# eth-cscs/conflux

Measured on NVIDIA H100. Metric: LU GFLOP/s (FP64, (2/3)N^3), higher is better.
Workload: dtype f64

## Files before the change

conflux_b200/__init__.py:

```python
import ctypes

import numpy as np

from ._lib import ConfluxError, LIB_PATH, SYMBOLS, check, lib

__all__ = ["pinned_empty", "pinned_free", "Comm", "lu_params", "LU_rep", "residual", "validate", "lu_solve", "lu_rcond", "lu_refine", "lu_equilibrate", "lu_svx", "lu_inverse", "lu_det", "timeline", "auto_grid", "lu_dims", "init_matrix_host", "ConfluxError", "dbg", "cholesky", "chol_dims", "chol_auto_grid"]


def auto_grid(M, N, P):
    px, py, pz = ctypes.c_int(), ctypes.c_int(), ctypes.c_int()
    check(lib().cflx_auto_grid(int(M), int(N), int(P), ctypes.byref(px), ctypes.byref(py), ctypes.byref(pz)), "auto_grid")
    return px.value, py.value, pz.value


def lu_dims(M, N, v, Px, Py, Pz):
    o = (ctypes.c_int * 8)()
    check(lib().cflx_lu_dims(int(M), int(N), int(v), int(Px), int(Py), int(Pz), o), "lu_dims")
    return dict(M=o[0], N=o[1], Ml=o[2], Nl=o[3], Nt=o[4], nlayr=o[5], Mt=o[6], P=o[7])


def init_matrix_host(M, N, v, Px, Py, Pz, rank, seed=42, out=None):
    d = lu_dims(M, N, v, Px, Py, Pz)
    if out is None:
        out = np.empty((d["Ml"], d["Nl"]), dtype=np.float64)
# ... 276 lines not shown
    def local_factor(self):
        L = np.empty((self.Ml, self.Nl))
        check(lib().cflx_chol_get_local(self._h, L.ctypes.data), "chol_get_local")
        return L

    def validate(self):
        a, r = ctypes.c_double(), ctypes.c_double()
        check(lib().cflx_chol_validate(self._h, ctypes.byref(a), ctypes.byref(r)), "chol_validate")
        return a.value, r.value

    def solve(self, B):
        B, B2, nrhs = _rhs(self.N, B, "cholesky.solve")
        X = np.empty_like(B2)
        check(lib().cflx_chol_solve(self._h, nrhs, B2.ctypes.data, max(nrhs, 1), X.ctypes.data, max(nrhs, 1)), "chol_solve")
        return X.reshape(B.shape)

    def rcond(self):
        r, a = ctypes.c_double(), ctypes.c_double()
        check(lib().cflx_chol_rcond(self._h, ctypes.byref(r), ctypes.byref(a)), "chol_rcond")
        return r.value, a.value

    def refine(self, B, X, ferr=True):
        shape, B2, X2, nrhs, fe, be = _refine_args(self.N, B, X, "cholesky.refine")
        check(lib().cflx_chol_refine(self._h, nrhs, B2.ctypes.data, nrhs, X2.ctypes.data, nrhs,
                                     fe.ctypes.data if ferr else None, be.ctypes.data), "chol_refine")
        return X2.reshape(shape), (fe if ferr else None), be

    def equilibrate(self, apply=True, upload=True):
        if upload:
            a = np.ascontiguousarray(self.data, dtype=np.float64)
            check(lib().cflx_chol_set_local(self._h, a.ctypes.data), "chol_set_local")
        s = np.zeros(self.N)
        scond, amax, equed, info = ctypes.c_double(), ctypes.c_double(), ctypes.c_char(), ctypes.c_int()
        check(lib().cflx_chol_equilibrate(self._h, 1 if apply else 0, s.ctypes.data, ctypes.byref(scond), ctypes.byref(amax),
                                          ctypes.byref(equed), ctypes.byref(info)), "chol_equilibrate")
        return dict(s=s, scond=scond.value, amax=amax.value, equed=equed.value.decode(), info=info.value)

    def svx(self, B):
        B, B2, nrhs = _rhs(self.N, B, "cholesky.svx")
        X = np.empty_like(B2)
        fe, be = np.empty(nrhs), np.empty(nrhs)
        rcond, equed, info = ctypes.c_double(), ctypes.c_char(), ctypes.c_int()
        check(lib().cflx_chol_svx(self._h, nrhs, B2.ctypes.data, nrhs, X.ctypes.data, nrhs, ctypes.byref(rcond),
                                  fe.ctypes.data, be.ctypes.data, ctypes.byref(equed), ctypes.byref(info)), "chol_svx")
        return X.reshape(B.shape), dict(rcond=rcond.value, ferr=fe, berr=be, equed=equed.value.decode(), info=info.value)

    def inverse(self, out=None):
        ptr, arr = _share_out(out, self.Ml, self.Nl, "cholesky.inverse")
        check(lib().cflx_chol_inverse(self._h, ptr), "chol_inverse")
        return arr

    def det(self, unscaled=False):
        ld, mant, exp = ctypes.c_double(), ctypes.c_double(), ctypes.c_int64()
        check(lib().cflx_chol_det(self._h, 1 if unscaled else 0, ctypes.byref(ld), ctypes.byref(mant), ctypes.byref(exp)),
              "chol_det")
        return dict(logdet=ld.value, mantissa=mant.value, exponent=exp.value)

    def finalize(self, clean=True):
        if self._h:
            lib().cflx_chol_destroy(self._h)
            self._h = ctypes.c_void_p()

    def __del__(self):
        try:
            self.finalize()
        except Exception:
            pass


def chol_dims(N, v, Px, Py, Pz):
    o = (ctypes.c_int * 6)()
    check(lib().cflx_chol_dims(int(N), int(v), int(Px), int(Py), int(Pz), o), "chol_dims")
    return dict(N=o[0], Kappa=o[1], Ml=o[2], Nl=o[3], l=o[4], P=o[5])


def chol_auto_grid(P, N):
    g = (ctypes.c_int * 3)()
    check(lib().cflx_chol_auto_grid(int(P), int(N), g), "chol_auto_grid")
    return tuple(g)


class dbg:

    @staticmethod
    def gemm_tn(AT, B, C=None, alpha=1.0, beta=0.0, reps=1):
        AT = np.asarray(AT, dtype=np.float64)
        B = np.asarray(B, dtype=np.float64)
        K, M = AT.shape
        N = B.shape[1]
        M2, N2 = M + (M & 1), N + (N & 1)
        ATp = np.zeros((K, M2))
        ATp[:, :M] = AT
        Bp = np.zeros((K, N2))
        Bp[:, :N] = B
        Cp = np.zeros((M, N2))
        if C is not None:
            Cp[:, :N] = C
        D, _, ms = dbg.gemm_tn_window(ATp, Bp, Cp, M, N2, K, alpha, beta, in_place=False, reps=reps)
        return D[:, :N], ms

    @staticmethod
    def gemm_tn_window(AT, B, C, M, N, K, alpha=1.0, beta=0.0, at_off=(0, 0), b_off=(0, 0), c_off=(0, 0), in_place=True,
                       reps=1):
        AT = np.ascontiguousarray(AT, dtype=np.float64)
        B = np.ascontiguousarray(B, dtype=np.float64)
        C = np.ascontiguousarray(C, dtype=np.float64)
        D = np.empty_like(C)
        Cout = D if in_place else np.empty_like(C)
        ms = ctypes.c_double()
        check(lib().cflx_dbg_gemm_tn(int(M), int(N), int(K), AT.ctypes.data, AT.shape[0], AT.shape[1],
                                     at_off[0] * AT.shape[1] + at_off[1], B.ctypes.data, B.shape[0], B.shape[1],
                                     b_off[0] * B.shape[1] + b_off[1], C.ctypes.data, C.shape[0], C.shape[1],
                                     int(c_off[0]), int(c_off[1]), float(alpha), float(beta), 1 if in_place else 0,
                                     D.ctypes.data, Cout.ctypes.data, int(reps), ctypes.byref(ms)), "dbg_gemm_tn")
        return D, Cout, ms.value

    @staticmethod
    def gemm_narrow(A, B, C=None, alpha=1.0, beta=0.0, reps=1, out=None):
        A = np.ascontiguousarray(A, dtype=np.float64)
        B = np.ascontiguousarray(B, dtype=np.float64)
        M, K = A.shape
        N = B.shape[1]
        Cp = None
        if C is not None:
            assert C.dtype == np.float64 and C.flags.c_contiguous and C.shape == (M, N)
            Cp = C.ctypes.data
        D = np.empty((M, N)) if out is None else out
        assert D.dtype == np.float64 and D.flags.c_contiguous and D.shape == (M, N)
        ms = ctypes.c_double()
        check(lib().cflx_dbg_gemm_narrow(M, N, K, A.ctypes.data, B.ctypes.data, Cp, float(alpha), float(beta), D.ctypes.data,
                                         int(reps), ctypes.byref(ms)), "dbg_gemm_narrow")
        return D, ms.value

    @staticmethod
    def gemm_narrow_tn(AT, B, C=None, alpha=1.0, beta=0.0, reps=1, out=None):
        AT = np.ascontiguousarray(AT, dtype=np.float64)
        B = np.ascontiguousarray(B, dtype=np.float64)
        K, M = AT.shape
        if B.ndim != 2 or B.shape[0] != K:
            raise ValueError(f"gemm_narrow_tn: B must have {K} rows, got shape {B.shape}")
        N = B.shape[1]
        Cp = None
        if C is not None:
            assert C.dtype == np.float64 and C.flags.c_contiguous and C.shape == (M, N)
            Cp = C.ctypes.data
        D = np.empty((M, N)) if out is None else out
        assert D.dtype == np.float64 and D.flags.c_contiguous and D.shape == (M, N)
        ms = ctypes.c_double()
        check(lib().cflx_dbg_gemm_narrow_tn(M, N, K, AT.ctypes.data, B.ctypes.data, Cp, float(alpha), float(beta),
                                            D.ctypes.data, int(reps), ctypes.byref(ms)), "dbg_gemm_narrow_tn")
        return D, ms.value

    @staticmethod
    def residual(A, mode, v, Kappa=None, grid=(1, 1), pos=(0, 0), Xc=None, Xr=None, reps=1):
        A = np.ascontiguousarray(A, dtype=np.float64)
        Ml, Nl = A.shape
        m = {"nn": 0, "tn": 1, "sym": 2}[mode]
        cvt = lambda X: None if X is None else np.ascontiguousarray(np.asarray(X, dtype=np.float64).reshape(X.shape[0], -1))
        Xc, Xr = cvt(Xc), cvt(Xr)
        nrhs = (Xc if Xc is not None else Xr).shape[1]
        rows = (Ml, Nl, Ml + Nl)[m]
        P, Q = np.empty((rows, nrhs)), np.empty((rows, nrhs))
        ms = ctypes.c_double()
        ptr = lambda a: a.ctypes.data if a is not None else None
        check(lib().cflx_dbg_residual(m, Ml, Nl, A.ctypes.data, int(v), int(Kappa if Kappa is not None else 1 << 30),
                                      int(grid[0]), int(grid[1]), int(pos[0]), int(pos[1]), nrhs, ptr(Xc), ptr(Xr),
                                      P.ctypes.data, Q.ctypes.data, int(reps), ctypes.byref(ms)), "dbg_residual")
        return P, Q, ms.value

    @staticmethod
    def equil(A, v, Kappa=None, grid=(1, 1), pos=(0, 0), M=None, r=None, c=None, equed="N", ncols=None):
        A = np.ascontiguousarray(A, dtype=np.float64)
        Ml, Nl = A.shape
        Px, Py = (int(x) for x in grid)
        M = int(M) if M is not None else (Ml // v) * Px * v
        r = np.ascontiguousarray(np.ones(M) if r is None else r, dtype=np.float64)
        c = np.ascontiguousarray(np.ones(M) if c is None else c, dtype=np.float64)
        out = dict(rowmax=np.empty(M), colmax=np.empty(M), diag=np.empty(M), scaled=np.empty_like(A),
                   sym_scaled=np.empty_like(A), growth=np.empty(2))
        zp = ctypes.c_int()
        check(lib().cflx_dbg_equil(Ml, Nl, int(v), int(Kappa if Kappa is not None else 1 << 30), Px, Py, int(pos[0]),
                                   int(pos[1]), M, A.ctypes.data, r.ctypes.data, c.ctypes.data, equed.encode(),
                                   int(ncols if ncols is not None else M), out["rowmax"].ctypes.data,
                                   out["colmax"].ctypes.data, out["diag"].ctypes.data, out["scaled"].ctypes.data,
                                   out["sym_scaled"].ctypes.data, out["growth"].ctypes.data, ctypes.byref(zp)), "dbg_equil")
        out["zero_pivot"] = zp.value
        return out

    @staticmethod
    def inverse_share(mode, v, grid, pos, M, c0, nc, Ml, Nl, Kappa=None, rows=None, X=None, perm=None, share=None,
                      zero_fill=False):
        m = {"lu": 0, "chol": 1}[mode]
        Px, Py = (int(x) for x in grid)
        ldn = -(-int(nc) // 8) * 8
        W = np.empty((Ml, ldn))
        ptr = lambda a: a.ctypes.data if a is not None else None
        out = Xc = pm = None
        if X is not None and share is not None:
            Xc = np.ascontiguousarray(X, dtype=np.float64)
            out = np.array(share, dtype=np.float64, order="C")
            pm = np.ascontiguousarray(perm, dtype=np.int32) if perm is not None else None
        check(lib().cflx_dbg_inverse_share(m, int(Ml), int(Nl), int(v), int(Kappa if Kappa is not None else 1 << 30), Px, Py,
                                           int(pos[0]), int(pos[1]), int(M), int(c0), int(nc),
                                           int(rows if rows is not None else Ml), ptr(Xc),
                                           Xc.shape[1] if Xc is not None else 0, ptr(pm), W.ctypes.data, ptr(out),
                                           1 if zero_fill else 0), "dbg_inverse_share")
        return W, out

    @staticmethod
    def det(d, s1=None, s2=None, square=False):
        d = np.ascontiguousarray(d, dtype=np.float64).ravel()
        n = d.size
        vec = lambda s: None if s is None else np.ascontiguousarray(s, dtype=np.float64).ravel()
        s1, s2 = vec(s1), vec(s2)
        for s in (s1, s2):
            if s is not None and s.size != n:
                raise ValueError(f"dbg.det: a divisor must have {n} entries, got {s.size}")
        mant, exp, neg, fz, nf = ctypes.c_double(), ctypes.c_int64(), ctypes.c_int(), ctypes.c_int(), ctypes.c_int()
        ptr = lambda a: a.ctypes.data if a is not None else None
        check(lib().cflx_dbg_det(n, d.ctypes.data, ptr(s1), ptr(s2), 1 if square else 0, ctypes.byref(mant),
                                 ctypes.byref(exp), ctypes.byref(neg), ctypes.byref(fz), ctypes.byref(nf)), "dbg_det")
        return dict(mantissa=mant.value, exponent=exp.value, neg=neg.value, first_zero=fz.value, nonfinite=nf.value)

    @staticmethod
    def panel(P, reps=1):
        P = np.ascontiguousarray(P, dtype=np.float64)
        n, v = P.shape
        perm = np.zeros(v, dtype=np.int32)
        A00 = np.zeros((v, v))
        LU = np.zeros((max(n, 1), v))
        ms = ctypes.c_double()
        check(lib().cflx_dbg_panel(n, v, P.ctypes.data, perm.ctypes.data, A00.ctypes.data, LU.ctypes.data, int(reps),
                                   ctypes.byref(ms)), "dbg_panel")
        return perm, A00, LU[:n], ms.value

    @staticmethod
    def trsm(A00, B=None, R=None, nb=0, ld=0):
        A00 = np.ascontiguousarray(A00, dtype=np.float64)
        v = A00.shape[0]
        X = Y = None
        n = B.shape[0] if B is not None else R.shape[1]
        if B is not None:
            B = np.ascontiguousarray(B, dtype=np.float64)
            X = np.empty_like(B)
        if R is not None:
            R = np.ascontiguousarray(R, dtype=np.float64)
            Y = np.empty_like(R)
        check(lib().cflx_dbg_trsm(n, v, int(nb), int(ld), A00.ctypes.data, B.ctypes.data if B is not None else None,
                                  X.ctypes.data if X is not None else None, R.ctypes.data if R is not None else None,
                                  Y.ctypes.data if Y is not None else None), "dbg_trsm")
        return X, Y

    @staticmethod
    def diag_inverse(A00, nb):
        A00 = np.ascontiguousarray(A00, dtype=np.float64)
        v = A00.shape[0]
        Uinv = np.empty((max(v // nb, 1), nb, nb))
        LinvT = np.empty_like(Uinv)
        check(lib().cflx_dbg_diag_inverse(v, int(nb), A00.ctypes.data, Uinv.ctypes.data, LinvT.ctypes.data), "dbg_diag_inverse")
        return Uinv, LinvT

    @staticmethod
    def potrf_tile(A, variant=0):
        A = np.ascontiguousarray(A, dtype=np.float64)
        v = A.shape[0]
        L = np.empty((v, v))
        LT = np.empty((v, v))
        info = ctypes.c_int()
        check(lib().cflx_dbg_potrf_tile(v, A.ctypes.data, L.ctypes.data, LT.ctypes.data, ctypes.byref(info), int(variant)),
              "dbg_potrf_tile")
        return L, LT, info.value

    @staticmethod
    def ozaki_gemm(AT, B, C=None, reps=1, want_planes=False, row0=0, col0=0, max_ctas=0):
        AT = np.ascontiguousarray(AT, dtype=np.float64)
        B = np.ascontiguousarray(B, dtype=np.float64)
        K, Ma = AT.shape
        Nb = B.shape[1]
        M, N = Ma - row0, Nb - col0
        D = np.empty((M, N))
        Cp = np.ascontiguousarray(C, dtype=np.float64) if C is not None else None
        pa = np.zeros((8, Ma, K), dtype=np.int8) if want_planes else None
        pb = np.zeros((8, Nb, K), dtype=np.int8) if want_planes else None
        ea = np.zeros(Ma, dtype=np.int32) if want_planes else None
        eb = np.zeros(Nb, dtype=np.int32) if want_planes else None
        ms, sms = ctypes.c_double(), ctypes.c_double()
        ptr = lambda a: a.ctypes.data if a is not None else None
        check(lib().cflx_dbg_ozaki_gemm(M, N, K, int(row0), int(col0), int(max_ctas), AT.ctypes.data, B.ctypes.data, ptr(Cp),
                                        D.ctypes.data, ptr(pa), ptr(pb), ptr(ea), ptr(eb), int(reps), ctypes.byref(ms),
                                        ctypes.byref(sms)), "dbg_ozaki_gemm")
        return dict(D=D, ms=ms.value, split_ms=sms.value, pa=pa, pb=pb, ea=ea, eb=eb)

    @staticmethod
    def push_pivots(A, pivot_rows, fnpr):
        A = np.array(A, dtype=np.float64, order="C")
        piv = np.ascontiguousarray(pivot_rows, dtype=np.int32)
        gri = np.zeros(A.shape[0], dtype=np.int32)
        a01 = np.zeros((max(1, len(piv)), A.shape[1]))
        check(lib().cflx_dbg_push_pivots(A.shape[0], A.shape[1], A.ctypes.data, len(piv), piv.ctypes.data, int(fnpr),
                                         gri.ctypes.data, a01.ctypes.data), "dbg_push_pivots")
        return A, gri, a01[:len(piv)]

    @staticmethod
    def wgmma_peak(n):
        t = ctypes.c_double()
        check(lib().cflx_dbg_wgmma_peak(int(n), ctypes.byref(t)), "dbg_wgmma_peak")
        return t.value

    @staticmethod
    def fp64_peak_ex(which):
        a, b = ctypes.c_double(), ctypes.c_double()
        check(lib().cflx_dbg_fp64_peak_ex(int(which), ctypes.byref(a), ctypes.byref(b)), "dbg_fp64_peak_ex")
        return a.value, b.value

    @staticmethod
    def fp64_peak(which):
        tf = ctypes.c_double()
        check(lib().cflx_dbg_fp64_peak(int(which), ctypes.byref(tf)), "dbg_fp64_peak")
        return tf.value
```

conflux_b200/_lib.py:

```python
import ctypes
import os

_HERE = os.path.dirname(os.path.abspath(__file__))
LIB_PATH = os.path.join(_HERE, "libconflux_b200.so")
_lib = None

c_double_p = ctypes.POINTER(ctypes.c_double)
c_int_p = ctypes.POINTER(ctypes.c_int)


class ConfluxError(RuntimeError):
    pass


SYMBOLS = [
    "cflx_last_error", "cflx_version", "cflx_device_count", "cflx_get_unique_id", "cflx_comm_create",
    "cflx_comm_barrier", "cflx_comm_destroy", "cflx_host_alloc", "cflx_host_free", "cflx_auto_grid", "cflx_lu_dims", "cflx_init_matrix_host",
    "cflx_lu_create", "cflx_lu_info", "cflx_lu_set_local", "cflx_lu_queue_next_local", "cflx_lu_factor", "cflx_lu_get_factors",
    "cflx_lu_get_permutation", "cflx_lu_residual", "cflx_lu_validate", "cflx_lu_solve", "cflx_lu_solve_trans", "cflx_lu_rcond", "cflx_lu_refine", "cflx_lu_equilibrate", "cflx_lu_svx", "cflx_lu_inverse", "cflx_lu_det", "cflx_lu_launch_count", "cflx_lu_uses_ozaki", "cflx_lu_set_profiling", "cflx_lu_phase_ms", "cflx_lu_timeline",
    "cflx_lu_set_kernel_timing", "cflx_lu_trailing_stats", "cflx_lu_destroy", "cflx_chol_auto_grid", "cflx_chol_auto_tile", "cflx_chol_dims", "cflx_chol_init_matrix_host",
    "cflx_chol_create", "cflx_chol_info", "cflx_chol_set_local", "cflx_chol_factor", "cflx_chol_get_local", "cflx_chol_validate",
    "cflx_chol_solve", "cflx_chol_rcond", "cflx_chol_refine", "cflx_chol_equilibrate", "cflx_chol_svx", "cflx_chol_inverse", "cflx_chol_det", "cflx_chol_launch_count", "cflx_chol_destroy", "cflx_dbg_gemm_tn", "cflx_dbg_gemm_narrow", "cflx_dbg_gemm_narrow_tn", "cflx_dbg_residual", "cflx_dbg_equil", "cflx_dbg_inverse_share", "cflx_dbg_det", "cflx_dbg_panel", "cflx_dbg_trsm", "cflx_dbg_diag_inverse", "cflx_dbg_potrf_tile", "cflx_dbg_push_pivots", "cflx_dbg_ozaki_gemm", "cflx_dbg_wgmma_peak", "cflx_dbg_fp64_peak", "cflx_dbg_fp64_peak_ex",
]


def _preload_nccl():
    import sys
    for d in sys.path:
        cand = os.path.join(d, "nvidia", "nccl", "lib", "libnccl.so.2")
        if os.path.exists(cand):
            try:
                ctypes.CDLL(cand, mode=ctypes.RTLD_GLOBAL)
                return cand
            except OSError:
                pass
    return None


def lib():
    global _lib
    if _lib is None:
        if not os.path.exists(LIB_PATH):
            raise ConfluxError(
                f"{LIB_PATH} is missing: build it with `python -c 'import __graft_entry__ as g; g.build()'` "
                "(conflux_b200 has no CPU fallback)")
        _preload_nccl()
        L = ctypes.CDLL(LIB_PATH)
        L.cflx_last_error.restype = ctypes.c_char_p
        L.cflx_version.restype = ctypes.c_char_p
        L.cflx_comm_destroy.restype = None
        L.cflx_lu_destroy.restype = None
        L.cflx_comm_destroy.argtypes = [ctypes.c_void_p]
        L.cflx_lu_destroy.argtypes = [ctypes.c_void_p]
        L.cflx_comm_barrier.argtypes = [ctypes.c_void_p]
        L.cflx_comm_create.argtypes = [ctypes.c_int, ctypes.c_int, ctypes.c_void_p, ctypes.c_int,
                                       ctypes.POINTER(ctypes.c_void_p)]
        L.cflx_lu_create.argtypes = [ctypes.c_void_p] + [ctypes.c_int] * 6 + [ctypes.POINTER(ctypes.c_void_p)]
        L.cflx_host_alloc.argtypes = [ctypes.c_size_t, ctypes.POINTER(ctypes.c_void_p)]
        L.cflx_host_free.argtypes = [ctypes.c_void_p]
        L.cflx_lu_info.argtypes = [ctypes.c_void_p, c_int_p]
        L.cflx_lu_set_local.argtypes = [ctypes.c_void_p, ctypes.c_void_p]
        L.cflx_lu_queue_next_local.argtypes = [ctypes.c_void_p, ctypes.c_void_p]
        L.cflx_lu_factor.argtypes = [ctypes.c_void_p, c_double_p]
        L.cflx_lu_get_factors.argtypes = [ctypes.c_void_p, ctypes.c_void_p, ctypes.c_void_p]
        L.cflx_lu_get_permutation.argtypes = [ctypes.c_void_p, ctypes.c_void_p]
        L.cflx_lu_residual.argtypes = [ctypes.c_void_p, c_double_p]
        L.cflx_lu_validate.argtypes = [ctypes.c_void_p, c_double_p, c_double_p]
        L.cflx_lu_solve.argtypes = [ctypes.c_void_p, ctypes.c_int, ctypes.c_void_p, ctypes.c_int, ctypes.c_void_p, ctypes.c_int]
        L.cflx_lu_solve_trans.argtypes = [ctypes.c_void_p, ctypes.c_int, ctypes.c_void_p, ctypes.c_int, ctypes.c_void_p,
                                          ctypes.c_int]
        L.cflx_lu_rcond.argtypes = [ctypes.c_void_p, c_double_p, c_double_p]
        L.cflx_lu_refine.argtypes = [ctypes.c_void_p, ctypes.c_int, ctypes.c_int, ctypes.c_void_p, ctypes.c_int, ctypes.c_void_p,
                                     ctypes.c_int, ctypes.c_void_p, ctypes.c_void_p]
        L.cflx_lu_equilibrate.argtypes = [ctypes.c_void_p, ctypes.c_int] + [ctypes.c_void_p] * 7
        L.cflx_lu_svx.argtypes = [ctypes.c_void_p, ctypes.c_int, ctypes.c_int, ctypes.c_void_p, ctypes.c_int, ctypes.c_void_p,
                                  ctypes.c_int] + [ctypes.c_void_p] * 6
        L.cflx_lu_inverse.argtypes = [ctypes.c_void_p, ctypes.c_void_p, c_int_p]
        L.cflx_lu_det.argtypes = [ctypes.c_void_p, ctypes.c_int] + [ctypes.c_void_p] * 5
        L.cflx_lu_uses_ozaki.argtypes = [ctypes.c_void_p]
        L.cflx_lu_launch_count.argtypes = [ctypes.c_void_p, ctypes.POINTER(ctypes.c_int64), ctypes.c_int]
        L.cflx_lu_set_profiling.argtypes = [ctypes.c_void_p, ctypes.c_int]
        L.cflx_lu_phase_ms.argtypes = [ctypes.c_void_p, c_double_p]
        L.cflx_lu_timeline.argtypes = [ctypes.c_void_p, ctypes.c_char_p, ctypes.c_int]
        L.cflx_lu_set_kernel_timing.argtypes = [ctypes.c_void_p, ctypes.c_int]
        L.cflx_lu_trailing_stats.argtypes = [ctypes.c_void_p, c_double_p, c_double_p]
        L.cflx_chol_destroy.restype = None
        L.cflx_chol_destroy.argtypes = [ctypes.c_void_p]
        L.cflx_chol_auto_grid.argtypes = [ctypes.c_int, ctypes.c_int, c_int_p]
        L.cflx_chol_auto_tile.argtypes = [ctypes.c_int] * 3
        L.cflx_chol_dims.argtypes = [ctypes.c_int] * 5 + [c_int_p]
        L.cflx_chol_init_matrix_host.argtypes = [ctypes.c_int] * 6 + [ctypes.c_void_p]
        L.cflx_chol_create.argtypes = [ctypes.c_void_p] + [ctypes.c_int] * 5 + [ctypes.POINTER(ctypes.c_void_p)]
        L.cflx_chol_info.argtypes = [ctypes.c_void_p, c_int_p]
        L.cflx_chol_set_local.argtypes = [ctypes.c_void_p, ctypes.c_void_p]
        L.cflx_chol_factor.argtypes = [ctypes.c_void_p, c_double_p]
        L.cflx_chol_get_local.argtypes = [ctypes.c_void_p, ctypes.c_void_p]
        L.cflx_chol_validate.argtypes = [ctypes.c_void_p, c_double_p, c_double_p]
        L.cflx_chol_solve.argtypes = [ctypes.c_void_p, ctypes.c_int, ctypes.c_void_p, ctypes.c_int, ctypes.c_void_p, ctypes.c_int]
        L.cflx_chol_rcond.argtypes = [ctypes.c_void_p, c_double_p, c_double_p]
        L.cflx_chol_refine.argtypes = [ctypes.c_void_p, ctypes.c_int, ctypes.c_void_p, ctypes.c_int, ctypes.c_void_p, ctypes.c_int,
                                       ctypes.c_void_p, ctypes.c_void_p]
        L.cflx_chol_equilibrate.argtypes = [ctypes.c_void_p, ctypes.c_int] + [ctypes.c_void_p] * 5
        L.cflx_chol_svx.argtypes = [ctypes.c_void_p, ctypes.c_int, ctypes.c_void_p, ctypes.c_int, ctypes.c_void_p, ctypes.c_int
                                    ] + [ctypes.c_void_p] * 5
        L.cflx_chol_inverse.argtypes = [ctypes.c_void_p, ctypes.c_void_p]
        L.cflx_chol_det.argtypes = [ctypes.c_void_p, ctypes.c_int] + [ctypes.c_void_p] * 3
        L.cflx_chol_launch_count.argtypes = [ctypes.c_void_p, ctypes.POINTER(ctypes.c_int64), ctypes.c_int]
        L.cflx_init_matrix_host.argtypes = [ctypes.c_int] * 8 + [ctypes.c_void_p]
        _buf = [ctypes.c_void_p, ctypes.c_int, ctypes.c_int64]
        L.cflx_dbg_gemm_tn.argtypes = [ctypes.c_int] * 3 + _buf + [ctypes.c_int64] + _buf + [ctypes.c_int64] + _buf + [
            ctypes.c_int] * 2 + [ctypes.c_double] * 2 + [ctypes.c_int, ctypes.c_void_p, ctypes.c_void_p, ctypes.c_int,
                                                          c_double_p]
        L.cflx_dbg_gemm_narrow.argtypes = [ctypes.c_int] * 3 + [ctypes.c_void_p] * 3 + [ctypes.c_double] * 2 + [
            ctypes.c_void_p, ctypes.c_int, c_double_p]
        L.cflx_dbg_gemm_narrow_tn.argtypes = [ctypes.c_int] * 3 + [ctypes.c_void_p] * 3 + [ctypes.c_double] * 2 + [
            ctypes.c_void_p, ctypes.c_int, c_double_p]
        L.cflx_dbg_residual.argtypes = [ctypes.c_int] * 3 + [ctypes.c_void_p] + [ctypes.c_int] * 7 + [ctypes.c_void_p] * 4 + [
            ctypes.c_int, c_double_p]
        L.cflx_dbg_equil.argtypes = [ctypes.c_int] * 9 + [ctypes.c_void_p] * 3 + [ctypes.c_char, ctypes.c_int] + [
            ctypes.c_void_p] * 7
        L.cflx_dbg_inverse_share.argtypes = [ctypes.c_int] * 13 + [ctypes.c_void_p, ctypes.c_int] + [ctypes.c_void_p] * 3 + [
            ctypes.c_int]
        L.cflx_dbg_det.argtypes = [ctypes.c_int] + [ctypes.c_void_p] * 3 + [ctypes.c_int] + [ctypes.c_void_p] * 5
        L.cflx_dbg_panel.argtypes = [ctypes.c_int, ctypes.c_int] + [ctypes.c_void_p] * 4 + [ctypes.c_int, c_double_p]
        L.cflx_dbg_trsm.argtypes = [ctypes.c_int] * 3 + [ctypes.c_int64] + [ctypes.c_void_p] * 5
        L.cflx_dbg_diag_inverse.argtypes = [ctypes.c_int, ctypes.c_int] + [ctypes.c_void_p] * 3
        L.cflx_dbg_potrf_tile.argtypes = [ctypes.c_int] + [ctypes.c_void_p] * 4 + [ctypes.c_int]
        L.cflx_dbg_push_pivots.argtypes = [ctypes.c_int, ctypes.c_int, ctypes.c_void_p, ctypes.c_int, ctypes.c_void_p, ctypes.c_int,
                                           ctypes.c_void_p, ctypes.c_void_p]
        L.cflx_dbg_ozaki_gemm.argtypes = [ctypes.c_int] * 6 + [ctypes.c_void_p] * 8 + [ctypes.c_int, c_double_p, c_double_p]
        L.cflx_dbg_wgmma_peak.argtypes = [ctypes.c_int, c_double_p]
        L.cflx_dbg_fp64_peak.argtypes = [ctypes.c_int, c_double_p]
        L.cflx_dbg_fp64_peak_ex.argtypes = [ctypes.c_int, c_double_p, c_double_p]
        _lib = L
    return _lib


def check(rc, what=""):
    if rc != 0:
        msg = lib().cflx_last_error().decode(errors="replace")
        raise ConfluxError(f"{what} failed with status {rc}: {msg}")
```

conflux_b200/csrc/dbg.cu:

```cuda
#include <algorithm>
#include <climits>
#include <limits>
#include <vector>

#include "../../include/conflux_b200.h"
#include "common.cuh"
#include "kernels.h"
#include "lu_state.h"

using namespace cflx;

namespace {
int check_device() {
    int n = 0;
    if (cudaGetDeviceCount(&n) != cudaSuccess || n == 0) {
        cudaGetLastError();
        set_last_error("no CUDA device visible: conflux_b200 has no CPU fallback");
        return CFLX_ERR_NO_DEVICE;
    }
    return CFLX_OK;
}

template <class Run>
int time_reps(Run&& run, int reps, double* ms_out) {
// ... 254 lines not shown
        CFLX_TRY(vec_out(colmax_out));
    }
    if (diag_out) {
        CFLX_TRY(equil_diag(a, L, vec, 0));
        CFLX_TRY(vec_out(diag_out));
    }
    if (scaled_out) {
        CFLX_CUDA(cudaMemcpy(w, a, sizeof(double) * a_n, cudaMemcpyDeviceToDevice));
        CFLX_TRY(equil_apply(w, L, dr.as<double>(), dc.as<double>(), equed, 0));
        CFLX_CUDA(cudaMemcpy(scaled_out, w, sizeof(double) * a_n, cudaMemcpyDeviceToHost));
    }
    if (sym_scaled_out) {
        CFLX_CUDA(cudaMemcpy(w, a, sizeof(double) * a_n, cudaMemcpyDeviceToDevice));
        CFLX_TRY(equil_sym_apply(w, L, dr.as<double>(), 0));
        CFLX_CUDA(cudaMemcpy(sym_scaled_out, w, sizeof(double) * a_n, cudaMemcpyDeviceToHost));
    }
    if (growth_out) {
        CFLX_TRY(equil_growth(a, a, L, ncols, dg.as<double>(), 0));
        CFLX_CUDA(cudaMemcpy(growth_out, dg.p, sizeof(double) * 2, cudaMemcpyDeviceToHost));
    }
    if (zero_pivot_out) {
        CFLX_TRY(equil_zero_pivot(a, L, dz.as<int>(), 0));
        int z = 0;
        CFLX_CUDA(cudaMemcpy(&z, dz.p, sizeof(int), cudaMemcpyDeviceToHost));
        *zero_pivot_out = z == INT_MAX ? 0 : z;
    }
    CFLX_CUDA(cudaDeviceSynchronize());
    return CFLX_OK;
}

int cflx_dbg_inverse_share(int mode, int Ml, int Nl, int v, int Kappa, int Px, int Py, int pi, int pj, int M, int c0,
                           int nc, int rows, const double* X, int ldx, const int* perm, double* W_out,
                           double* share_inout, int zero_fill) {
    CFLX_TRY(check_device());
    if ((mode != 0 && mode != 1) || Ml < 0 || Nl < 0 || v < 1 || Ml % v || Nl % v || Px < 1 || Py < 1 || pi < 0 ||
        pi >= Px || pj < 0 || pj >= Py || M < (Ml / v) * Px * v || M < (Nl / v) * Py * v || c0 < 0 || nc < 1 ||
        c0 + nc > M || rows < 0 || rows > Ml || (share_inout && (!X || ldx < nc || (mode == 0 && !perm))))
        return CFLX_ERR_ARG;
    const Layout L{M, v, Kappa, Ml, Nl, Px, Py, pi, pj};
    const int ldn = (int)round_up(nc, 8);
    if (W_out) {
        DevBuf dW;
        CFLX_TRY(dW.alloc(sizeof(double) * Ml * ldn));
        CFLX_CUDA(cudaMemset(dW.p, 0, sizeof(double) * Ml * ldn));
        CFLX_TRY(launch_inverse_seed(dW.as<double>(), ldn, L, rows, c0, nc, 0));
        CFLX_CUDA(cudaMemcpy(W_out, dW.p, sizeof(double) * Ml * ldn, cudaMemcpyDeviceToHost));
    }
    if (share_inout) {
        const size_t a_n = (size_t)Ml * Nl;
        DevBuf dA, dX, dp;
        CFLX_TRY(dA.alloc(sizeof(double) * a_n));
        CFLX_TRY(dX.alloc(sizeof(double) * M * ldx));
        CFLX_TRY(dp.alloc(sizeof(int) * M));
        CFLX_CUDA(cudaMemcpy(dA.p, share_inout, sizeof(double) * a_n, cudaMemcpyHostToDevice));
        CFLX_CUDA(cudaMemcpy(dX.p, X, sizeof(double) * M * ldx, cudaMemcpyHostToDevice));
        if (mode == 0) CFLX_CUDA(cudaMemcpy(dp.p, perm, sizeof(int) * M, cudaMemcpyHostToDevice));
        CFLX_TRY(launch_inverse_scatter(mode == 0 ? InvKind::LU : InvKind::Chol, dX.as<double>(), ldx, c0, nc,
                                        mode == 0 ? dp.as<int>() : nullptr, L, dA.as<double>(), 0));
        if (mode == 1 && zero_fill) CFLX_TRY(launch_inverse_zero(L, dA.as<double>(), 0));
        CFLX_CUDA(cudaMemcpy(share_inout, dA.p, sizeof(double) * a_n, cudaMemcpyDeviceToHost));
    }
    CFLX_CUDA(cudaDeviceSynchronize());
    return CFLX_OK;
}

int cflx_dbg_det(int n, const double* d, const double* s1, const double* s2, int square, double* mant_out,
                 int64_t* exp_out, int* neg_out, int* first_zero_out, int* nonfinite_out) {
    CFLX_TRY(check_device());
    if (n < 1 || !d || (square != 0 && square != 1)) return CFLX_ERR_ARG;
    DevBuf dv, dr;
    CFLX_TRY(dv.alloc(sizeof(double) * 3 * (size_t)n));
    CFLX_TRY(dr.alloc(sizeof(DetResult)));
    double* v = dv.as<double>();
    CFLX_CUDA(cudaMemcpy(v, d, sizeof(double) * n, cudaMemcpyHostToDevice));
    if (s1) CFLX_CUDA(cudaMemcpy(v + n, s1, sizeof(double) * n, cudaMemcpyHostToDevice));
    if (s2) CFLX_CUDA(cudaMemcpy(v + 2 * (size_t)n, s2, sizeof(double) * n, cudaMemcpyHostToDevice));
    CFLX_TRY(launch_det(v, s1 ? v + n : nullptr, s2 ? v + 2 * (size_t)n : nullptr, n, square != 0, dr.as<DetResult>(), 0));
    DetResult r{};
    CFLX_CUDA(cudaMemcpy(&r, dr.p, sizeof(r), cudaMemcpyDeviceToHost));
    if (mant_out) *mant_out = r.mant;
    if (exp_out) *exp_out = r.exp;
    if (neg_out) *neg_out = r.neg;
    if (first_zero_out) *first_zero_out = r.first_zero;
    if (nonfinite_out) *nonfinite_out = r.nonfinite;
    return CFLX_OK;
}

int cflx_dbg_residual(int mode, int Ml, int Nl, const double* A, int v, int Kappa, int Px, int Py, int pi, int pj,
                      int nrhs, const double* Xc, const double* Xr, double* P_out, double* Q_out, int reps, double* ms_out) {
    CFLX_TRY(check_device());
    if (mode < 0 || mode > 2 || Ml < 0 || Nl < 0 || (Nl & 1) || v < 4 || (v & 3) || nrhs < 1 || !A || Px < 1 || Py < 1 ||
        pi < 0 || pi >= Px || pj < 0 || pj >= Py || (mode != 1 && !Xc) || (mode != 0 && !Xr))
        return CFLX_ERR_ARG;
    const ResidMode m = mode == 0 ? ResidMode::NN : mode == 1 ? ResidMode::TN : ResidMode::SymLower;
    const int rows = mode == 0 ? Ml : mode == 1 ? Nl : Ml + Nl;
    const size_t a_n = (size_t)Ml * Nl, o_n = (size_t)std::max(rows, 1) * nrhs;
    DevBuf dA, dXc, dXr, dP, dQ;
    CFLX_TRY(dA.alloc(sizeof(double) * a_n));
    CFLX_TRY(dXc.alloc(sizeof(double) * (size_t)Nl * nrhs));
    CFLX_TRY(dXr.alloc(sizeof(double) * (size_t)Ml * nrhs));
    CFLX_TRY(dP.alloc(sizeof(double) * o_n));
    CFLX_TRY(dQ.alloc(sizeof(double) * o_n));
    CFLX_CUDA(cudaMemcpy(dA.p, A, sizeof(double) * a_n, cudaMemcpyHostToDevice));
    if (Xc) CFLX_CUDA(cudaMemcpy(dXc.p, Xc, sizeof(double) * (size_t)Nl * nrhs, cudaMemcpyHostToDevice));
    if (Xr) CFLX_CUDA(cudaMemcpy(dXr.p, Xr, sizeof(double) * (size_t)Ml * nrhs, cudaMemcpyHostToDevice));
    const Layout L{0, v, Kappa, Ml, Nl, Px, Py, pi, pj};
    auto run = [&]() {
        return launch_residual(m, dA.as<double>(), L, dXc.as<double>(), dXr.as<double>(), nrhs, nrhs, dP.as<double>(),
                               dQ.as<double>(), nrhs, 0);
    };
    CFLX_TRY(time_reps(run, reps, ms_out));
    CFLX_CUDA(cudaMemset(dP.p, 0, sizeof(double) * o_n));
    CFLX_CUDA(cudaMemset(dQ.p, 0, sizeof(double) * o_n));
    CFLX_TRY(run());
    if (P_out) CFLX_CUDA(cudaMemcpy(P_out, dP.p, sizeof(double) * (size_t)rows * nrhs, cudaMemcpyDeviceToHost));
    if (Q_out) CFLX_CUDA(cudaMemcpy(Q_out, dQ.p, sizeof(double) * (size_t)rows * nrhs, cudaMemcpyDeviceToHost));
    CFLX_CUDA(cudaDeviceSynchronize());
    return CFLX_OK;
}

int cflx_dbg_panel(int n, int v, const double* panel, int* perm_out, double* A00_out, double* LU_out, int reps,
                   double* ms_out) {
    CFLX_TRY(check_device());
    if (n < 0 || v <= 0) return CFLX_ERR_ARG;
    const int64_t ld = std::max<int64_t>(2, round_up(n, 2));
    std::vector<double> WT((size_t)v * ld, 0.0);
    for (int r = 0; r < n; ++r)
        for (int c = 0; c < v; ++c) WT[(size_t)c * ld + r] = panel[(size_t)r * v + c];
    DevBuf dW, dW0, dA00, dA00T, dperm;
    CFLX_TRY(dW.alloc(sizeof(double) * v * ld));
    CFLX_TRY(dW0.alloc(sizeof(double) * v * ld));
    CFLX_TRY(dA00.alloc(sizeof(double) * v * v));
    CFLX_TRY(dA00T.alloc(sizeof(double) * v * v));
    CFLX_TRY(dperm.alloc(sizeof(int) * 2 * v));
    CFLX_CUDA(cudaMemcpy(dW0.p, WT.data(), sizeof(double) * v * ld, cudaMemcpyHostToDevice));
    CFLX_CUDA(cudaMemset(dA00.p, 0, sizeof(double) * v * v));
    Events<2> ev;
    CFLX_TRY(ev.create());
    PanelWorkspace ws{};
    CFLX_TRY(panel_workspace_create(&ws));
    if (const char* e = getenv("CFLX_PANEL_CTAS")) ws.cta_cap = atoi(e);
    if (reps < 1) reps = 1;
    float total = 0;
    int nb = 0, rc = CFLX_OK;
    for (int r = 0; r < reps + 1 && rc == CFLX_OK; ++r) {
        cudaMemcpyAsync(dW.p, dW0.p, sizeof(double) * v * ld, cudaMemcpyDeviceToDevice, 0);
        cudaEventRecord(ev[0]);
        rc = launch_panel_getrf_a00(dW.as<double>(), ld, n, v, dperm.as<int>(), dA00.as<double>(), &nb, &ws, 0);
        cudaEventRecord(ev[1]);
        if (cudaEventSynchronize(ev[1]) != cudaSuccess) rc = CFLX_ERR_CUDA;
        float ms = 0;
        cudaEventElapsedTime(&ms, ev[0], ev[1]);
        if (r > 0) total += ms;
    }
    if (rc == CFLX_OK && n >= v)
        rc = launch_gather_a00(dW.as<double>(), ld, dperm.as<int>(), v, nb, dA00.as<double>(), dA00T.as<double>(), 0);
    panel_workspace_destroy(&ws);
    if (rc != CFLX_OK) {
        if (rc == CFLX_ERR_CUDA) set_last_error("panel kernel failed: %s", cudaGetErrorString(cudaGetLastError()));
        return rc;
    }
    if (ms_out) *ms_out = total / reps;
    if (perm_out) CFLX_CUDA(cudaMemcpy(perm_out, dperm.p, sizeof(int) * v, cudaMemcpyDeviceToHost));
    if (A00_out) CFLX_CUDA(cudaMemcpy(A00_out, dA00.p, sizeof(double) * v * v, cudaMemcpyDeviceToHost));
    if (LU_out) {
        CFLX_CUDA(cudaMemcpy(WT.data(), dW.p, sizeof(double) * v * ld, cudaMemcpyDeviceToHost));
        for (int r = 0; r < n; ++r)
            for (int c = 0; c < v; ++c) LU_out[(size_t)r * v + c] = WT[(size_t)c * ld + r];
    }
    CFLX_CUDA(cudaDeviceSynchronize());
    return CFLX_OK;
}

int cflx_dbg_trsm(int n, int v, int nb, int64_t ld, const double* A00, const double* B, double* X_out, const double* R,
                  double* Y_out) {
    CFLX_TRY(check_device());
    if (n <= 0 || v <= 0 || v % 4 != 0) return CFLX_ERR_ARG;
    if (nb == 0)
        for (int c : {128, 64, 32, 16, 8, 4})
            if (!nb && v % c == 0) nb = c;
    if (nb != 4 && nb != 8 && nb != 16 && nb != 32 && nb != 64 && nb != 128) return CFLX_ERR_UNSUPPORTED;
    if (v % nb != 0) return CFLX_ERR_ARG;
    if (ld == 0) ld = round_up(n, 2);
    if ((ld & 1) || ld < round_up(n, 2)) return CFLX_ERR_ARG;
    const double nan = std::numeric_limits<double>::quiet_NaN();
    std::vector<double> A00T((size_t)v * v), BT((size_t)v * ld, nan), RT((size_t)v * ld, nan);
    for (int i = 0; i < v; ++i)
        for (int j = 0; j < v; ++j) A00T[(size_t)j * v + i] = A00[(size_t)i * v + j];
    DevBuf dA, dAT, dUinv, dLinvT, dP, dL, dR, dU;
    CFLX_TRY(dA.alloc(8 * (size_t)v * v)); CFLX_TRY(dAT.alloc(8 * (size_t)v * v));
    CFLX_TRY(dUinv.alloc(8 * (size_t)v * v)); CFLX_TRY(dLinvT.alloc(8 * (size_t)v * v));
    CFLX_TRY(dP.alloc(8 * (size_t)v * ld)); CFLX_TRY(dL.alloc(8 * (size_t)v * ld));
    CFLX_TRY(dR.alloc(8 * (size_t)v * ld)); CFLX_TRY(dU.alloc(8 * (size_t)v * ld));
    CFLX_CUDA(cudaMemcpy(dA.p, A00, 8 * (size_t)v * v, cudaMemcpyHostToDevice));
    CFLX_CUDA(cudaMemcpy(dAT.p, A00T.data(), 8 * (size_t)v * v, cudaMemcpyHostToDevice));
    CFLX_TRY(launch_diag_inverses(dA.as<double>(), v, nb, dUinv.as<double>(), dLinvT.as<double>(), 0));
    if (B && X_out) {
        for (int r = 0; r < n; ++r)
            for (int c = 0; c < v; ++c) BT[(size_t)c * ld + r] = B[(size_t)r * v + c];
        CFLX_CUDA(cudaMemcpy(dP.p, BT.data(), 8 * (size_t)v * ld, cudaMemcpyHostToDevice));
        CFLX_CUDA(cudaMemset(dL.p, 0, 8 * (size_t)v * ld));
        CFLX_TRY(trsm_right_upper_T(dA.as<double>(), dUinv.as<double>(), v, nb, dP.as<double>(), dL.as<double>(), ld, n, 0));
        CFLX_CUDA(cudaMemcpy(BT.data(), dL.p, 8 * (size_t)v * ld, cudaMemcpyDeviceToHost));
        for (int r = 0; r < n; ++r)
            for (int c = 0; c < v; ++c) X_out[(size_t)r * v + c] = BT[(size_t)c * ld + r];
    }
    if (R && Y_out) {
        for (int i = 0; i < v; ++i)
            for (int c = 0; c < n; ++c) RT[(size_t)i * ld + c] = R[(size_t)i * n + c];
        CFLX_CUDA(cudaMemcpy(dR.p, RT.data(), 8 * (size_t)v * ld, cudaMemcpyHostToDevice));
        CFLX_CUDA(cudaMemset(dU.p, 0, 8 * (size_t)v * ld));
        CFLX_TRY(trsm_left_lower_unit(dAT.as<double>(), dLinvT.as<double>(), v, nb, dR.as<double>(), dU.as<double>(), ld,
                                      (int)round_up(n, 2), 0));
        CFLX_CUDA(cudaMemcpy(RT.data(), dU.p, 8 * (size_t)v * ld, cudaMemcpyDeviceToHost));
        for (int i = 0; i < v; ++i)
            for (int c = 0; c < n; ++c) Y_out[(size_t)i * n + c] = RT[(size_t)i * ld + c];
    }
    CFLX_CUDA(cudaDeviceSynchronize());
    return CFLX_OK;
}

int cflx_dbg_diag_inverse(int v, int nb, const double* A00, double* Uinv_out, double* LinvT_out) {
    CFLX_TRY(check_device());
    if (v <= 0 || nb <= 0 || v % nb != 0 || !A00) return CFLX_ERR_ARG;
    const size_t vv = (size_t)v * v, blocks = (size_t)v * nb;
    DevBuf dA, dU, dL;
    CFLX_TRY(dA.alloc(8 * vv));
    CFLX_TRY(dU.alloc(8 * blocks));
    CFLX_TRY(dL.alloc(8 * blocks));
    CFLX_CUDA(cudaMemcpy(dA.p, A00, 8 * vv, cudaMemcpyHostToDevice));
    CFLX_TRY(launch_diag_inverses(dA.as<double>(), v, nb, dU.as<double>(), dL.as<double>(), 0));
    if (Uinv_out) CFLX_CUDA(cudaMemcpy(Uinv_out, dU.p, 8 * blocks, cudaMemcpyDeviceToHost));
    if (LinvT_out) CFLX_CUDA(cudaMemcpy(LinvT_out, dL.p, 8 * blocks, cudaMemcpyDeviceToHost));
    CFLX_CUDA(cudaDeviceSynchronize());
    return CFLX_OK;
}

int cflx_dbg_potrf_tile(int v, const double* A, double* L_out, double* LT_out, int* info_out, int variant) {
    CFLX_TRY(check_device());
    if (!A || v < 4 || v > 512 || variant < 0 || variant > 2 || (variant == 1 && v != 128) ||
        (variant == 2 && potrf_tile_scratch(v) == 0))
        return CFLX_ERR_ARG;
    const size_t vv = (size_t)v * v;
    DevBuf dD, dUT, dUc, dQ, dinfo;
    CFLX_TRY(dD.alloc(8 * vv));
    CFLX_TRY(dUT.alloc(8 * vv));
    CFLX_TRY(dUc.alloc(8 * vv));
    CFLX_TRY(dinfo.alloc(sizeof(int)));
    if (variant == 2) CFLX_TRY(dQ.alloc(8 * potrf_tile_scratch(v)));
    CFLX_CUDA(cudaMemcpy(dD.p, A, 8 * vv, cudaMemcpyHostToDevice));
    CFLX_CUDA(cudaMemset(dUT.p, 0, 8 * vv));
    CFLX_CUDA(cudaMemset(dinfo.p, 0, sizeof(int)));
    CFLX_TRY(potrf_setup(v));
    int64_t launches = 0;
    if (variant == 1)
        CFLX_TRY(potrf_block128(dD.as<double>(), v, dUT.as<double>(), v, dUc.as<double>(), dinfo.as<int>(), 0, 0));
    else
        CFLX_TRY(potrf_tile(dD.as<double>(), dUT.as<double>(), dQ.as<double>(), dinfo.as<int>(), 0, v, 0, &launches));
    if (L_out) CFLX_CUDA(cudaMemcpy(L_out, dD.p, 8 * vv, cudaMemcpyDeviceToHost));
    if (LT_out) CFLX_CUDA(cudaMemcpy(LT_out, dUT.p, 8 * vv, cudaMemcpyDeviceToHost));
    if (info_out) CFLX_CUDA(cudaMemcpy(info_out, dinfo.p, sizeof(int), cudaMemcpyDeviceToHost));
    CFLX_CUDA(cudaDeviceSynchronize());
    return CFLX_OK;
}

int cflx_dbg_push_pivots(int n_rows, int n_cols, double* A_inout, int npiv, const int* pivot_rows, int fnpr, int* gri_out,
                         double* a01_out) {
    CFLX_TRY(check_device());
    if (n_rows <= 0 || n_cols <= 0 || (n_cols & 1) || npiv < 0 || npiv > n_rows - fnpr || fnpr < 0) return CFLX_ERR_ARG;
    if (npiv == 0) {
        if (gri_out) for (int i = 0; i < n_rows; ++i) gri_out[i] = i;
        return CFLX_OK;
    }
    const int v = npiv;
    DevBuf dA, dtmp, da01, dplan, dgp, dgri, dgrit, digri;
    CFLX_TRY(dA.alloc(8 * (size_t)n_rows * n_cols));
    CFLX_TRY(dtmp.alloc(8 * (size_t)v * n_cols));
    CFLX_TRY(da01.alloc(8 * (size_t)v * n_cols));
    CFLX_TRY(dplan.alloc(sizeof(int) * (6 * (size_t)v + 8 + n_rows)));
    CFLX_TRY(dgp.alloc(sizeof(int) * v));
    CFLX_TRY(dgri.alloc(sizeof(int) * n_rows));
    CFLX_TRY(dgrit.alloc(sizeof(int) * n_rows));
    CFLX_TRY(digri.alloc(sizeof(int) * n_rows));
    CFLX_CUDA(cudaMemcpy(dA.p, A_inout, 8 * (size_t)n_rows * n_cols, cudaMemcpyHostToDevice));
    CFLX_CUDA(cudaMemcpy(dgp.p, pivot_rows, sizeof(int) * v, cudaMemcpyHostToDevice));
    MovePlan plan{};
    int* pm = dplan.as<int>();
    plan.npiv = pm; plan.nel = pm + 4; pm += 8;
    plan.cur_piv = pm; pm += v;
    plan.order = pm; pm += v;
    plan.slot2piv = pm; pm += v;
    plan.early = pm; pm += v;
    plan.late = pm; pm += 2 * v;
    plan.rowsrc = pm;
    CFLX_TRY(launch_iota_gri(dgri.as<int>(), digri.as<int>(), n_rows, n_rows, 1, 0, 0));
    CFLX_TRY(launch_plan_moves(dgp.as<int>(), v, 1, 0, fnpr, n_rows, digri.as<int>(), plan, 0));
    CFLX_TRY(launch_push_phase1(dA.as<double>(), n_cols, n_cols, 0, plan, v, dtmp.as<double>(), da01.as<double>(), n_cols, 0, 0));
    CFLX_TRY(launch_push_phase2(dA.as<double>(), n_cols, n_cols, 0, plan, v, 0));
    CFLX_TRY(launch_push_phase3(dA.as<double>(), n_cols, n_cols, 0, fnpr, plan, v, dtmp.as<double>(), 0));
    CFLX_TRY(launch_update_gri(dgri.as<int>(), dgrit.as<int>(), digri.as<int>(), plan.rowsrc, fnpr, n_rows, n_rows, 1, 0));
    CFLX_CUDA(cudaMemcpy(A_inout, dA.p, 8 * (size_t)n_rows * n_cols, cudaMemcpyDeviceToHost));
    if (gri_out) CFLX_CUDA(cudaMemcpy(gri_out, dgri.p, sizeof(int) * n_rows, cudaMemcpyDeviceToHost));
    if (a01_out) CFLX_CUDA(cudaMemcpy(a01_out, da01.p, 8 * (size_t)v * n_cols, cudaMemcpyDeviceToHost));
    CFLX_CUDA(cudaDeviceSynchronize());
    return CFLX_OK;
}

int cflx_dbg_ozaki_gemm(int M, int N, int K, int row0, int col0, int max_ctas, const double* AT, const double* B,
                        const double* C, double* D, signed char* planesA_out, signed char* planesB_out, int* ea_out,
                        int* eb_out, int reps, double* ms_out, double* split_ms_out) {
    CFLX_TRY(check_device());
    if (M <= 0 || N <= 0 || K <= 0 || (N & 1) || row0 < 0 || col0 < 0 || max_ctas < 0) return CFLX_ERR_ARG;
    const int Ma = row0 + M, Nb = col0 + N;
    const int64_t ldat = round_up(Ma, 2), ldb = Nb, ldc = N;
    DevBuf dA, dB, dC, dC0;
    CFLX_TRY(dA.alloc(sizeof(double) * K * ldat));
    CFLX_TRY(dB.alloc(sizeof(double) * K * ldb));
    CFLX_TRY(dC.alloc(sizeof(double) * M * ldc));
    CFLX_TRY(dC0.alloc(sizeof(double) * M * ldc));
    CFLX_CUDA(cudaMemset(dA.p, 0, sizeof(double) * K * ldat));
    CFLX_CUDA(cudaMemcpy2D(dA.p, ldat * 8, AT, (size_t)Ma * 8, (size_t)Ma * 8, K, cudaMemcpyHostToDevice));
    CFLX_CUDA(cudaMemcpy(dB.p, B, sizeof(double) * K * ldb, cudaMemcpyHostToDevice));
    if (C) CFLX_CUDA(cudaMemcpy(dC0.p, C, sizeof(double) * M * ldc, cudaMemcpyHostToDevice));
    else CFLX_CUDA(cudaMemset(dC0.p, 0, sizeof(double) * M * ldc));
    Events<3> ev;
    CFLX_TRY(ev.create());
    OzakiWorkspace ws;
    int rc = ozaki_workspace_create(&ws, Ma, Nb, K);
    if (reps < 1) reps = 1;
    float ms = 0, ms_split = 0;
    for (int r = 0; r < reps + 1 && rc == CFLX_OK; ++r) {
        cudaMemcpyAsync(dC.p, dC0.p, sizeof(double) * M * ldc, cudaMemcpyDeviceToDevice, 0);
        cudaEventRecord(ev[0]);
        rc = ozaki_split_a(&ws, dA.as<double>(), ldat, Ma, 0);
        if (!rc && col0 > 0) rc = ozaki_split_b(&ws, dB.as<double>(), ldb, 0, col0, 0);
        if (!rc) rc = ozaki_split_b(&ws, dB.as<double>(), ldb, col0, N, 0);
        cudaEventRecord(ev[1]);
        if (!rc) rc = launch_ozaki_gemm(&ws, M, N, row0, col0, dC.as<double>(), ldc, max_ctas, 0);
        cudaEventRecord(ev[2]);
        if (cudaEventSynchronize(ev[2]) != cudaSuccess) {
            set_last_error("ozaki kernel failed: %s", cudaGetErrorString(cudaGetLastError()));
            rc = CFLX_ERR_CUDA;
        }
        float a = 0, b = 0;
        cudaEventElapsedTime(&a, ev[0], ev[1]);
        cudaEventElapsedTime(&b, ev[1], ev[2]);
        if (r > 0) {
            ms_split += a;
            ms += b;
        }
    }
    if (rc == CFLX_OK) {
        if (D) cudaMemcpy(D, dC.p, sizeof(double) * M * ldc, cudaMemcpyDeviceToHost);
        for (int s = 0; s < 8; ++s) {
            if (planesA_out) cudaMemcpy(planesA_out + (size_t)s * Ma * K, ws.planesA + (size_t)s * ws.cap_a * K, (size_t)Ma * K, cudaMemcpyDeviceToHost);
            if (planesB_out) cudaMemcpy(planesB_out + (size_t)s * Nb * K, ws.planesB + (size_t)s * ws.cap_b * K, (size_t)Nb * K, cudaMemcpyDeviceToHost);
        }
        if (ea_out) cudaMemcpy(ea_out, ws.ea, sizeof(int) * Ma, cudaMemcpyDeviceToHost);
        if (eb_out) cudaMemcpy(eb_out, ws.eb, sizeof(int) * Nb, cudaMemcpyDeviceToHost);
        if (cudaDeviceSynchronize() != cudaSuccess) rc = CFLX_ERR_CUDA;
    }
    ozaki_workspace_destroy(&ws);
    if (ms_out) *ms_out = ms / reps;
    if (split_ms_out) *split_ms_out = ms_split / reps;
    return rc;
}

int cflx_dbg_wgmma_peak(int n, double* tmacs_out) {
    CFLX_TRY(check_device());
    if (!tmacs_out) return CFLX_ERR_ARG;
    return wgmma_peak_probe(n, tmacs_out);
}

}
```

conflux_b200/csrc/gemm.cu:

```cuda
#include <cstdlib>

#include "common.cuh"
#include "kernels.h"

namespace cflx {

namespace {
constexpr int BK = 16, STAGES = 4;

template <int WM, int WN>
struct Cfg {
    static constexpr int BM = 64 * WM, BN = 32 * WN;
    static constexpr int LDA = BM + 4, LDB = BN + 4;
    static constexpr int NCONS = WM * WN, NTHREADS = (NCONS + 1) * 32;
    static constexpr bool STAGE_C = (WM == 2);
    static constexpr int NBAR = 2 * STAGES + (STAGE_C ? WM * STAGES : 0);
    static constexpr size_t SMEM = (size_t)STAGES * BK * (LDA + LDB) * sizeof(double) + NBAR * sizeof(uint64_t);
    static_assert(!STAGE_C || (LDA == LDB && 64 / 16 == STAGES), "one slab per warp row and stage, in both parts");
};

__device__ __forceinline__ double2 ld_c2(const double* p) {
    double2 v;
    asm("ld.global.v2.f64 {%0, %1}, [%2];" : "=d"(v.x), "=d"(v.y) : "l"(p));
    return v;
}

template <int WM, int WN, int MINB>
__global__ void __launch_bounds__(Cfg<WM, WN>::NTHREADS, MINB) gemm_tn_kernel(GemmArgs g) {
    using C = Cfg<WM, WN>;
    constexpr int BM = C::BM, BN = C::BN, LDA = C::LDA, LDB = C::LDB, NCONS = C::NCONS;
    extern __shared__ __align__(128) unsigned char smem_raw[];
    double* sA = reinterpret_cast<double*>(smem_raw);
    double* sB = sA + STAGES * BK * LDA;
    uint64_t* full = reinterpret_cast<uint64_t*>(sB + STAGES * BK * LDB);
    uint64_t* empty = full + STAGES;
    uint64_t* cfull = empty + STAGES;

    const int warp = threadIdx.x >> 5, lane = threadIdx.x & 31;
    const int m0 = blockIdx.y * BM, n0 = blockIdx.x * BN;

    if (threadIdx.x == 0) {
        for (int s = 0; s < STAGES; ++s) {
            mbar_init(&full[s], 1);
            mbar_init(&empty[s], NCONS);
        }
        if constexpr (C::STAGE_C)
            for (int b = 0; b < WM * STAGES; ++b) mbar_init(&cfull[b], 1);
        fence_barrier_init();
    }
    __syncthreads();

    if (warp == NCONS) {
        int wm = g.M - m0;
        wm = wm > BM ? BM : ((wm + 1) & ~1);
        int wn = g.N - n0;
        wn = wn > BN ? BN : ((wn + 1) & ~1);
        const int rr = lane & 15;
        const int nkt = (g.K + BK - 1) / BK;
        const bool use_c = (g.beta != 0.0);
        for (int kt = 0; kt < nkt; ++kt) {
            const int s = kt % STAGES, u = kt / STAGES;
            if (u > 0) mbar_wait(&empty[s], (u - 1) & 1);
            const int rows = min(BK, g.K - kt * BK);
            if (lane == 0) mbar_arrive_expect_tx(&full[s], (uint32_t)(rows * (wm + wn) * sizeof(double)));
            __syncwarp();
            if (rr < rows) {
                const int64_t k = (int64_t)kt * BK + rr;
                if (lane < 16)
                    bulk_g2s(sA + (s * BK + rr) * LDA, g.AT + k * g.ldat + m0, (uint32_t)(wm * sizeof(double)), &full[s]);
                else
                    bulk_g2s(sB + (s * BK + rr) * LDB, g.B + k * g.ldb + n0, (uint32_t)(wn * sizeof(double)), &full[s]);
            }
        }
        if constexpr (C::STAGE_C) {
            if (use_c)
                for (int i = 0; i < STAGES; ++i) {
                    const int s = (nkt + i) % STAGES, kt = nkt + i - STAGES;
                    if (kt >= 0) mbar_wait(&empty[s], (kt / STAGES) & 1);
                    const int wr = lane >> 4, r0 = m0 + 64 * wr + 16 * i;
                    const int rows = max(0, min(16, g.M - r0));
                    uint64_t* bar = &cfull[wr * STAGES + i];
                    if (rr == 0) mbar_arrive_expect_tx(bar, (uint32_t)(rows * wn * sizeof(double)));
                    __syncwarp();
                    if (rr < rows)
                        bulk_g2s(sA + (wr * STAGES + s) * BK * LDA + rr * LDA + 4 * (rr & 1),
                                 g.C + (int64_t)(r0 + rr) * g.ldc + n0, (uint32_t)(wn * sizeof(double)), bar);
                }
        }
        return;
    }

    const int wm_off = (warp / WN) * 64, wn_off = (warp % WN) * 32;
    const int g4 = lane >> 2, t4 = lane & 3;
    double acc[4][4][4];
#pragma unroll
    for (int i = 0; i < 4; ++i)
#pragma unroll
        for (int j = 0; j < 4; ++j) acc[i][j][0] = acc[i][j][1] = acc[i][j][2] = acc[i][j][3] = 0.0;

    int kt = 0;
    for (; kt * BK < g.K; ++kt) {
        const int s = kt % STAGES, u = kt / STAGES;
        mbar_wait(&full[s], u & 1);
        const double* a_s = sA + s * BK * LDA + wm_off + g4;
        const double* b_s = sB + s * BK * LDB + wn_off + g4;
        const int rows = min(BK, g.K - kt * BK);
#pragma unroll
        for (int kk = 0; kk < BK; kk += 8) {
            if (kk < rows) {
                const bool hi = kk + 4 < rows;
                const double* a_k = a_s + (kk + t4) * LDA;
                const double* b_k = b_s + (kk + t4) * LDB;
                double b[4][2];
#pragma unroll
                for (int j = 0; j < 4; ++j) {
                    b[j][0] = b_k[8 * j];
                    b[j][1] = hi ? b_k[4 * LDB + 8 * j] : 0.0;
                }
#pragma unroll
                for (int i = 0; i < 4; ++i) {
                    const double a[4] = {a_k[16 * i], a_k[16 * i + 8], hi ? a_k[4 * LDA + 16 * i] : 0.0,
                                         hi ? a_k[4 * LDA + 16 * i + 8] : 0.0};
#pragma unroll
                    for (int j = 0; j < 4; ++j) dmma16x8x8(acc[i][j], a, b[j]);
                }
            }
        }
        __syncwarp();
        if (lane == 0) mbar_arrive(&empty[s]);
    }

    const double alpha = g.alpha, beta = g.beta;
    const bool use_c = (beta != 0.0);
    const int row0 = m0 + wm_off + g4, col0 = n0 + wn_off + 2 * t4;
    if constexpr (C::STAGE_C) {
        const int wr = warp / WN, nkt = kt;
#pragma unroll
        for (int i = 0; i < 4; ++i) {
            const double* cs = sA + (wr * STAGES + (nkt + i) % STAGES) * BK * LDA + 4 * (g4 & 1) + wn_off + 2 * t4;
            if (use_c) mbar_wait(&cfull[wr * STAGES + i], 0);
#pragma unroll
            for (int h = 0; h < 2; ++h) {
                const int row = row0 + 16 * i + 8 * h;
#pragma unroll
                for (int j = 0; j < 4; ++j) {
                    const int col = col0 + 8 * j;
                    if (row < g.M && col < g.N) {
                        double2 cv = make_double2(0.0, 0.0);
                        if (use_c) cv = *reinterpret_cast<const double2*>(cs + (g4 + 8 * h) * LDA + 8 * j);
                        double2 out;
                        out.x = fma(alpha, acc[i][j][2 * h], beta * cv.x);
                        out.y = fma(alpha, acc[i][j][2 * h + 1], beta * cv.y);
                        *reinterpret_cast<double2*>(g.D + (int64_t)row * g.ldd + col) = out;
                    }
                }
            }
        }
    } else {
#pragma unroll
        for (int sl = 0; sl < 8; ++sl) {
            const int row = row0 + 8 * sl;
            double2 cv[4];
#pragma unroll
            for (int j = 0; j < 4; ++j) {
                const int col = col0 + 8 * j;
                cv[j] = make_double2(0.0, 0.0);
                if (use_c && row < g.M && col < g.N) cv[j] = ld_c2(g.C + (int64_t)row * g.ldc + col);
            }
#pragma unroll
            for (int j = 0; j < 4; ++j) {
                const int col = col0 + 8 * j;
                if (row < g.M && col < g.N) {
                    double2 out;
                    out.x = fma(alpha, acc[sl / 2][j][2 * (sl & 1)], beta * cv[j].x);
                    out.y = fma(alpha, acc[sl / 2][j][2 * (sl & 1) + 1], beta * cv[j].y);
                    *reinterpret_cast<double2*>(g.D + (int64_t)row * g.ldd + col) = out;
                }
            }
        }
    }
}
}

namespace {
template <int WM, int WN, int MINB>
int setup_one() {
    static PerDeviceMax cfg;
    if (cfg.raise(Cfg<WM, WN>::SMEM))
        CFLX_CUDA(cudaFuncSetAttribute(gemm_tn_kernel<WM, WN, MINB>, cudaFuncAttributeMaxDynamicSharedMemorySize,
                                       (int)Cfg<WM, WN>::SMEM));
    return CFLX_OK;
}
template <int WM, int WN, int MINB>
int launch_one(const GemmArgs& g, cudaStream_t stream) {
    using C = Cfg<WM, WN>;
    CFLX_TRY((setup_one<WM, WN, MINB>()));
    dim3 grid((g.N + C::BN - 1) / C::BN, (g.M + C::BM - 1) / C::BM);
    gemm_tn_kernel<WM, WN, MINB><<<grid, C::NTHREADS, C::SMEM, stream>>>(g);
    CFLX_CUDA(cudaGetLastError());
    return CFLX_OK;
}
int tile_variant() {
    static int v = -1;
    if (v < 0) {
        const char* e = getenv("CFLX_GEMM_TILE");
        v = (e && atoi(e) == 64) ? 64 : 128;
    }
    return v;
}
}

int gemm_tn_setup() {
    CFLX_TRY((setup_one<2, 4, 1>()));
    CFLX_TRY((setup_one<1, 4, 2>()));
    return CFLX_OK;
}

int launch_gemm_tn(const GemmArgs& g, cudaStream_t stream) {
    if (g.M <= 0 || g.N <= 0 || g.K <= 0) return CFLX_OK;
    if ((g.K & 3) || (g.N & 1) || (g.ldat & 1) || (g.ldb & 1) || (g.ldc & 1) || (g.ldd & 1)) {
        set_last_error("gemm_tn: unsupported shape M=%d N=%d K=%d ld=(%lld,%lld,%lld,%lld)", g.M, g.N, g.K,
                       (long long)g.ldat, (long long)g.ldb, (long long)g.ldc, (long long)g.ldd);
        return CFLX_ERR_UNSUPPORTED;
    }
    if (tile_variant() == 64) return launch_one<1, 4, 2>(g, stream);
    return launch_one<2, 4, 1>(g, stream);
}

}
```

conflux_b200/csrc/kernels.h:

```cpp
#pragma once
#include <cuda_runtime.h>

#include <cstdint>

namespace cflx {

struct GemmArgs {
    int M, N, K;
    const double* AT;
    int64_t ldat;
    const double* B;
    int64_t ldb;
    const double* C;
    int64_t ldc;
    double* D;
    int64_t ldd;
    double alpha, beta;
};
int gemm_tn_setup();
int launch_gemm_tn(const GemmArgs& g, cudaStream_t stream);

struct OzakiWorkspace {
    struct Maps;
    int8_t* planesA = nullptr;
    int8_t* planesB = nullptr;
    int* ea = nullptr;
    int* eb = nullptr;
    Maps* maps = nullptr;
    int K = 0, cap_a = 0, cap_b = 0, sms = 0;
};
int ozaki_workspace_create(OzakiWorkspace* ws, int max_rows, int max_cols, int K);
void ozaki_workspace_destroy(OzakiWorkspace* ws);
int ozaki_split_a(OzakiWorkspace* ws, const double* LT, int64_t ld, int n, cudaStream_t s);
int ozaki_split_b(OzakiWorkspace* ws, const double* U, int64_t ld, int col0, int n, cudaStream_t s);
int wgmma_peak_probe(int n, double* tmacs_out);
int launch_ozaki_gemm(OzakiWorkspace* ws, int M, int N, int row0, int col0, double* C, int64_t ldc, int max_ctas, cudaStream_t s);

struct PanelWorkspace {
    void* slot_hdr;
    void* slot_rows;
    int epoch;
    int max_ctas;
    int cta_cap;
    unsigned* sk_flags;
    int* sk_ppos;
    unsigned* sk_ticket;
    unsigned sk_epoch, sk_ticket_count;
    int sk_enabled;
};
int panel_workspace_create(PanelWorkspace* ws);
void panel_workspace_destroy(PanelWorkspace* ws);
int launch_panel_getrf(double* W, int64_t ldw, int n, int v, int* perm_out, PanelWorkspace* ws, cudaStream_t stream);
int launch_panel_getrf_a00(double* W, int64_t ldw, int n, int v, int* perm_out, double* A00, int* nb_used,
                           PanelWorkspace* ws, cudaStream_t stream);

int launch_extract_panel_T(const double* A, int64_t lda, int64_t row0, int64_t col0, int n, int v, double* PT,
                           int64_t ldp, cudaStream_t stream);
int launch_store_panel_T(double* A, int64_t lda, int64_t row0, int64_t col0, int n, int v, const double* LT,
                         int64_t ldp, cudaStream_t stream);
int launch_gather_winners(const double* PT, int64_t ldp, const int* tags, int n_valid, const int* perm, int v,
                          double* out_vals, int64_t ldo, int* out_tags, int dst0, cudaStream_t stream);
int launch_gather_a00(const double* W, int64_t ldw, const int* perm, int v, int nb, double* A00, double* A00T,
                      cudaStream_t stream);

struct MovePlan {
    int* npiv;
    int* cur_piv;
    int* order;
    int* slot2piv;
    int* early;
    int* late;
    int* nel;
    int* rowsrc;
};
int launch_plan_moves(const int* gpivots, int v, int Px, int pi, int fnpr, int Ml, const int* igri, MovePlan plan,
                      cudaStream_t stream);
int launch_push_phase1(const double* A, int64_t lda, int ncols, int col_lo, MovePlan plan, int v, double* tmp,
                       double* a01raw, int64_t ld01, int c0, cudaStream_t stream);
int launch_push_phase2(double* A, int64_t lda, int ncols, int col_lo, MovePlan plan, int v, cudaStream_t stream);
int launch_push_phase3(double* A, int64_t lda, int ncols, int col_lo, int fnpr, MovePlan plan, int v,
                       const double* tmp, cudaStream_t stream);
int launch_update_gri(int* gri, int* gri_tmp, int* igri, const int* rowsrc, int fnpr, int Ml, int v, int Px,
                      cudaStream_t stream);
int launch_compact_panel(const double* PT, int64_t ldp, double* PT2, int64_t ldp2, const int* rowsrc, int fnpr_old,
                         const int* npiv, int Ml, int v, cudaStream_t stream);
int launch_store_u_rows(double* A, int64_t lda, int fnpr_old, MovePlan plan, const double* U, int64_t ldu, int c0,
                        int ncols, int v, cudaStream_t stream);
int launch_store_diag(double* A, int64_t lda, int fnpr_old, MovePlan plan, const double* A00, int loff, int v,
                      cudaStream_t stream);
int launch_split_factors(const double* F, int64_t ldf, int n, double* LT, double* U, cudaStream_t stream);
int launch_gather_perm_rows(const double* A, int64_t lda, const int* perm, int n, double* out, cudaStream_t stream);
constexpr int SUMSQ_PARTIALS = 1184;
int launch_sumsq(const double* X, int64_t count, double* out, double* partials, cudaStream_t stream);
int launch_sum_partials(const double* partials, int n, double* out, cudaStream_t stream);
int launch_fill(double* p, int64_t n, double val, cudaStream_t stream);
int launch_iota_gri(int* gri, int* igri, int Ml, int v, int Px, int pi, cudaStream_t stream);
int launch_pack_bcast(const double* A00, const int* tags, int v, double* buf, cudaStream_t stream);
int launch_unpack_bcast(const double* buf, int v, double* A00, double* A00T, int* gpivots, cudaStream_t stream);
int launch_record_pivots(const int* gpivots, int v, int* hist, int k, cudaStream_t stream);

int launch_diag_inverses(const double* A00, int v, int nb, double* Uinv, double* LinvT, cudaStream_t stream);
int trsm_right_upper_T(const double* A00, const double* Uinv, int v, int nb, double* PT, double* LT, int64_t ld,
                       int n, cudaStream_t stream);
int trsm_left_lower_unit(const double* A00T, const double* LinvT, int v, int nb, double* R, double* U, int64_t ld,
                         int n, cudaStream_t stream);

size_t potrf_tile_scratch(int v);
int potrf_setup(int v);
int potrf_tile(double* D, double* UT, double* Q, int* info, int col0, int v, cudaStream_t stream, int64_t* launches);
int potrf_block128(double* D, int ldd, double* UT, int ldu, double* Uc, int* info, int col0, cudaStream_t stream);

int launch_gather_rows(const double* A, int64_t lda, const int* src_rows, int nrows, int ncols, double* out,
                       cudaStream_t stream);

int launch_gemm_narrow(int M, int N, int K, const double* A, int64_t lda, const double* B, int64_t ldb, const double* C,
                       int64_t ldc, double* D, int64_t ldd, double alpha, double beta, cudaStream_t stream);
int launch_gemm_narrow_tn(int M, int N, int K, const double* AT, int64_t ldat, const double* B, int64_t ldb,
                          const double* C, int64_t ldc, double* D, int64_t ldd, double alpha, double beta,
                          cudaStream_t stream);

enum class ResidMode { NN, TN, SymLower };

}
```

conflux_b200/csrc/lu.cu:

```cuda
#include <algorithm>
#include <cmath>
#include <cstdarg>
#include <cstdlib>
#include <cstring>
#include <random>
#include <string>
#include <vector>

#include <nvtx3/nvToolsExt.h>

#include "lu_state.h"

namespace cflx {
static thread_local char g_err[1024] = "";
void set_last_error(const char* fmt, ...) {
    va_list ap;
    va_start(ap, fmt);
    vsnprintf(g_err, sizeof(g_err), fmt, ap);
    va_end(ap);
}
}

using namespace cflx;

namespace {
int flipbit(int n, int k) { return n ^ (1 << k); }
int butterfly_pair(int pi, int r, int Px) {
    int src = flipbit(pi, r);
    if (src >= Px) {
        if (r == 0) src = pi;
        else {
            src = flipbit(src, r - 1);
            if (src >= Px) src = Px - 1;
        }
    }
    return src;
}
#include "init_tables.inc"
bool fixed_input_matrix(int n, std::vector<double>* out) {
    for (const InitTable& t : kInitTables) {
        if (t.n != n) continue;
        out->clear();
        out->reserve((size_t)n * n);
        if (t.kind == 0) {
            for (const char* p = t.text; *p; ++p) out->push_back((double)(*p - '0'));
        } else {
            const char* p = t.text;
            while (*p) {
                char* e = nullptr;
                out->push_back(std::strtod(p, &e));
                p = (*e == ',') ? e + 1 : e;
            }
        }
        return out->size() == (size_t)n * n;
    }
    return false;
}
int pick_nb(int v) {
    static int cap = -1;
    if (cap < 0) {
        const char* e = getenv("CFLX_TRSM_NB");
        cap = e ? atoi(e) : 128;
    }
    for (int nb : {128, 64, 32, 16, 8, 4})
        if (nb <= cap && v % nb == 0) return nb;
    return 0;
}
}

namespace cflx {
int make_sub(cflx_comm* c, int color, int key, int size, SubComm* out) {
    out->size = size;
    out->rank = key;
    out->c = nullptr;
    if (c->world_size == 1) return CFLX_OK;
    CFLX_NCCL(ncclCommSplit(c->world, color, key, &out->c, nullptr));
    int r = -1, s = -1;
    CFLX_NCCL(ncclCommUserRank(out->c, &r));
    CFLX_NCCL(ncclCommCount(out->c, &s));
    if (r != key || s != size) {
        set_last_error("sub-communicator mismatch: rank %d/%d expected %d/%d", r, s, key, size);
        return CFLX_ERR_NCCL;
    }
    return CFLX_OK;
}
int grid_barrier(cflx_comm* c) {
    if (c->world_size > 1)
        CFLX_NCCL(ncclAllReduce(c->d_scratch, c->d_scratch, 1, ncclDouble, ncclSum, c->world, c->stream));
    CFLX_CUDA(cudaStreamSynchronize(c->stream));
    return CFLX_OK;
}
int grid_init(Grid* g, cflx_comm* c, int Px, int Py, int Pz) {
    g->comm = c;
    g->Px = Px; g->Py = Py; g->Pz = Pz; g->P = Px * Py * Pz;
    g->rank = c->world_rank;
    g->pi = g->rank / (Py * Pz);
    g->pj = (g->rank / Pz) % Py;
    g->pk = g->rank % Pz;
    CFLX_TRY(make_sub(c, g->pi * Py + g->pj, g->pk, Pz, &g->k_comm));
    return make_sub(c, g->pj * Pz + g->pk, g->pi, Px, &g->i_comm);
}
void grid_free(Grid* g) {
    for (SubComm* sc : {&g->k_comm, &g->i_comm})
        if (sc->c) ncclCommDestroy(sc->c);
}

int handle_init(Handle* h, const HandleTexts* texts, cflx_comm* c, int Px, int Py, int Pz) {
    h->texts = texts;
    CFLX_TRY(grid_init(h, c, Px, Py, Pz));
    CFLX_TRY(dmalloc(&h->A0, (size_t)h->Ml * h->Nl));
    return dmalloc(&h->A11, (size_t)h->Ml * h->Nl);
}
int handle_update_setup(Handle* h) {
    CFLX_TRY(gemm_tn_setup());
    const char* e = getenv("CFLX_GEMM");
    if (e && !strcmp(e, "ozaki") && h->nlayr % 128 == 0 && h->nlayr <= 512) {
        CFLX_TRY(ozaki_workspace_create(&h->oz, h->Ml, h->Nl, h->nlayr));
        h->use_ozaki = true;
    }
    return CFLX_OK;
}
int handle_side_stream(Handle* h) {
    int lo = 0, hi = 0;
    cudaDeviceGetStreamPriorityRange(&lo, &hi);
    CFLX_CUDA(cudaStreamCreateWithPriority(&h->side, cudaStreamNonBlocking, hi));
    return CFLX_OK;
}
void handle_free(Handle* h) {
    cudaFree(h->A0);
    cudaFree(h->A11);
    solve_cache_free(&h->sv);
    equil_free(&h->eq);
    if (h->use_ozaki) ozaki_workspace_destroy(&h->oz);
    if (h->side) cudaStreamDestroy(h->side);
    grid_free(h);
}
int handle_set_local(Handle* h, const double* host_local) {
    CFLX_CUDA(cudaSetDevice(h->comm->device));
    cudaStream_t s = h->comm->stream;
    CFLX_CUDA(cudaMemcpyAsync(h->A0, host_local, (size_t)h->Ml * h->Nl * sizeof(double), cudaMemcpyHostToDevice, s));
    CFLX_CUDA(cudaStreamSynchronize(s));
    h->have_input = true;
    h->factored = false;
    h->sv.ready = false;
    h->eq.in.equed = 'N';
    return CFLX_OK;
}
int handle_check(const Handle* h, const char* what) {
    if (h->factored) return CFLX_OK;
    set_last_error(h->texts->unfactored, what);
    return CFLX_ERR_STATE;
}
int handle_equil_begin(Handle* h, bool apply) {
    if (!h->have_input) {
        set_last_error("%s", h->texts->no_input);
        return CFLX_ERR_STATE;
    }
    if (apply && h->eq.in.equed != 'N') {
        set_last_error(h->texts->scaled, h->eq.in.equed);
        return CFLX_ERR_STATE;
    }
    CFLX_CUDA(cudaSetDevice(h->comm->device));
    h->factored = false;
    h->sv.ready = false;
    return CFLX_OK;
}
int handle_equil_end(Handle* h, bool apply, int info, char equed, double rowcnd, double colcnd, const double* c) {
    if (apply && info == 0) CFLX_TRY(equil_record_set(&h->eq.in, equed, rowcnd, colcnd, h->eq.qr, c, h->M, h->comm->stream));
    return CFLX_OK;
}
int handle_launch_count(Handle* h, int64_t* count_out, int reset) {
    if (!h || !count_out) return CFLX_ERR_ARG;
    *count_out = h->launches;
    if (reset) h->launches = 0;
    return CFLX_OK;
}
}

namespace {
struct PhaseTimer {
    cflx_lu* lu;
    int rg;
    cudaStream_t st;
    cudaEvent_t a = nullptr, b = nullptr;
    int ev = -1;
    PhaseTimer(cflx_lu* l, int region, cudaStream_t stream) : lu(l), rg(region), st(stream) {
        nvtxRangePushA(region_name(rg));
        if (lu->prof_mode == 1) {
            cudaEventCreate(&a);
            cudaEventCreate(&b);
            cudaEventRecord(a, st);
        } else if (lu->prof_mode == 2) {
            ev = (int)lu->tl_recs.size() * 2;
            while ((int)lu->tl_pool.size() < ev + 2) {
                cudaEvent_t e;
                cudaEventCreate(&e);
                lu->tl_pool.push_back(e);
            }
            lu->tl_recs.push_back({rg, st == lu->comm->stream ? 0 : 1, ev});
            cudaEventRecord(lu->tl_pool[ev], st);
        }
    }
    ~PhaseTimer() {
        if (lu->prof_mode == 1) {
            cudaEventRecord(b, st);
            cudaEventSynchronize(b);
            float ms = 0;
            cudaEventElapsedTime(&ms, a, b);
            lu->phase_ms[region_phase(rg)] += ms;
            lu->region_ms[st == lu->comm->stream ? 0 : 1][rg] += ms;
            lu->region_cnt[st == lu->comm->stream ? 0 : 1][rg]++;
            cudaEventDestroy(a);
            cudaEventDestroy(b);
        } else if (lu->prof_mode == 2) {
            cudaEventRecord(lu->tl_pool[ev + 1], st);
        }
        nvtxRangePop();
    }
};

int tournament_exchange(cflx_lu* lu, int r, int my_half, cudaStream_t s) {
    const int v = lu->v, Px = lu->Px, pi = lu->pi;
    const int src = butterfly_pair(pi, r, Px);
    const int other = 1 - my_half;
    const size_t hv = (size_t)v * v;
    double* mine = lu->candH + my_half * hv;
    double* recv = lu->candH + other * hv;
    int* mine_t = lu->tagsH + my_half * v;
    int* recv_t = lu->tagsH + other * v;
    const bool self = (src == pi);
    if (self) {
        CFLX_CUDA(cudaMemcpyAsync(recv, mine, hv * sizeof(double), cudaMemcpyDeviceToDevice, s));
        CFLX_CUDA(cudaMemcpyAsync(recv_t, mine_t, v * sizeof(int), cudaMemcpyDeviceToDevice, s));
    }
    bool any = !self;
    for (int ppi = 0; ppi < Px && !any; ++ppi) any = (ppi != pi && butterfly_pair(ppi, r, Px) == pi);
    if (!any) return CFLX_OK;
    CFLX_NCCL(ncclGroupStart());
    for (int ppi = 0; ppi < Px; ++ppi) {
        if (ppi == pi || butterfly_pair(ppi, r, Px) != pi) continue;
        const bool mutual = (!self && ppi == src);
        const double* sv = mutual ? mine : lu->candH + hv;
        const int* st = mutual ? mine_t : lu->tagsH + v;
        CFLX_NCCL(ncclSend(sv, hv, ncclDouble, ppi, lu->i_comm.c, s));
        CFLX_NCCL(ncclSend(st, v, ncclInt, ppi, lu->i_comm.c, s));
    }
    if (!self) {
        CFLX_NCCL(ncclRecv(recv, hv, ncclDouble, src, lu->i_comm.c, s));
        CFLX_NCCL(ncclRecv(recv_t, v, ncclInt, src, lu->i_comm.c, s));
    }
    CFLX_NCCL(ncclGroupEnd());
    return CFLX_OK;
}

__global__ void stack_kernel(const double* __restrict__ candH, const int* __restrict__ tagsH, int v, double* __restrict__ S,
                             double* __restrict__ W2, int* __restrict__ tagsS) {
    const int64_t e = (int64_t)blockIdx.x * blockDim.x + threadIdx.x;
    const int64_t tot = (int64_t)2 * v * v;
    if (e < tot) {
        const int c = (int)(e / (2 * v)), hi = (int)(e % (2 * v));
        const int h = hi / v, i = hi % v;
        const double x = candH[(size_t)h * v * v + (size_t)c * v + i];
        S[e] = x;
        W2[e] = x;
    }
    if (e < 2 * v) tagsS[e] = tagsH[e];
}
int panel_phase(cflx_lu* lu, int k, int fnpr, cudaStream_t s) {
    const int v = lu->v, Px = lu->Px, Py = lu->Py, Pz = lu->Pz, Ml = lu->Ml, Nl = lu->Nl;
    const int pi = lu->pi, pj = lu->pj, pk = lu->pk;
    const int loff = (k / Py) * v, pjk = k % Py;
    if (pj != pjk) return CFLX_OK;
    double* A00 = lu->A00 + (size_t)(k & 1) * v * v;
    double* A00T = lu->A00T + (size_t)(k & 1) * v * v;
    const int n_old = Ml - fnpr;
    const int64_t ldk = std::max<int64_t>(2, round_up(n_old, 2));
    int nR = 0;
    while ((1 << nR) < Px) ++nR;
    {
        PhaseTimer t(lu, RG_step0_copy, s);
        CFLX_TRY(launch_extract_panel_T(lu->A11, Nl, fnpr, loff, n_old, v, lu->PT, ldk, s));
        lu->launches++;
    }
    if (Pz > 1 && n_old > 0) {
        PhaseTimer t(lu, RG_step0_reduce, s);
        CFLX_NCCL(ncclReduce(lu->PT, lu->PT, (size_t)v * ldk, ncclDouble, ncclSum, 0, lu->k_comm.c, s));
    }
    if (pk != 0) return CFLX_OK;
    int my_half = 0;
    {
        PhaseTimer t(lu, RG_step1_A10copy, s);
        CFLX_CUDA(cudaMemcpyAsync(lu->W, lu->PT, (size_t)v * ldk * sizeof(double), cudaMemcpyDeviceToDevice, s));
    }
    {
        PhaseTimer t(lu, RG_step1_lup, s);
        int nb_used = 0;
        if (nR == 0) {
            CFLX_TRY(launch_panel_getrf_a00(lu->W, ldk, n_old, v, lu->perm, A00, &nb_used, &lu->pws, s));
            CFLX_TRY(launch_gather_a00(lu->W, ldk, lu->perm, v, nb_used, A00, A00T, s));
            lu->launches += 2;
        } else {
            CFLX_TRY(launch_panel_getrf(lu->W, ldk, n_old, v, lu->perm, &lu->pws, s));
            lu->launches++;
        }
    }
    {
        PhaseTimer t(lu, RG_step1_rowpermute, s);
        int first_partner = flipbit(pi, 0);
        if (first_partner > Px - 1) first_partner = Px - 1;
        my_half = first_partner < pi ? 1 : 0;
        CFLX_TRY(launch_gather_winners(lu->PT, ldk, lu->gri + fnpr, n_old, lu->perm, v,
                                       lu->candH + (size_t)my_half * v * v, v, lu->tagsH + my_half * v, 0, s));
        lu->launches++;
    }
    PhaseTimer t(lu, RG_step1_pivoting, s);
    for (int r = 0; r < nR; ++r) {
        CFLX_TRY(tournament_exchange(lu, r, my_half, s));
        const int64_t tot = (int64_t)2 * v * v;
        stack_kernel<<<(unsigned)((tot + 255) / 256), 256, 0, s>>>(lu->candH, lu->tagsH, v, lu->S, lu->W2, lu->tagsS);
        CFLX_CUDA(cudaGetLastError());
        const bool last = (r == nR - 1);
        int nb_used = 0;
        if (last) {
            CFLX_TRY(launch_panel_getrf_a00(lu->W2, 2 * v, 2 * v, v, lu->perm, A00, &nb_used, &lu->pws, s));
            CFLX_TRY(launch_gather_a00(lu->W2, 2 * v, lu->perm, v, nb_used, A00, A00T, s));
            lu->launches++;
            my_half = 0;
        } else {
            CFLX_TRY(launch_panel_getrf(lu->W2, 2 * v, 2 * v, v, lu->perm, &lu->pws, s));
            my_half = butterfly_pair(pi, r + 1, Px) < pi ? 1 : 0;
        }
        CFLX_TRY(launch_gather_winners(lu->S, 2 * v, lu->tagsS, 2 * v, lu->perm, v, lu->candH + (size_t)my_half * v * v,
                                       v, lu->tagsH + my_half * v, 0, s));
        lu->launches += 3;
    }
    return CFLX_OK;
}

int ozaki_planes_a(cflx_lu* lu, int n_act, int64_t ld2, cudaStream_t s) {
    if (!lu->use_ozaki || n_act <= 0) return CFLX_OK;
    PhaseTimer t(lu, RG_step6_dgemm, s);
    lu->launches++;
    return ozaki_split_a(&lu->oz, lu->LT + (int64_t)lu->pk * lu->nlayr * ld2, ld2, n_act, s);
}
int ozaki_planes_b(cflx_lu* lu, int col0, int n, int64_t ldu, cudaStream_t s) {
    if (!lu->use_ozaki || n <= 0) return CFLX_OK;
    PhaseTimer t(lu, RG_step6_dgemm, s);
    lu->launches++;
    return ozaki_split_b(&lu->oz, lu->U + (int64_t)lu->pk * lu->nlayr * ldu, ldu, col0, n, s);
}

int trailing_gemm(cflx_lu* lu, int k, int part, int fnpr, int n_act, int col_lo, int ncols, int64_t ld2, int64_t ldu,
                  int u_col_off, cudaStream_t s, int max_ctas = 0) {
    if (n_act <= 0 || ncols <= 0) return CFLX_OK;
    PhaseTimer t(lu, RG_step6_dgemm, s);
    GemmArgs g{};
    g.M = n_act;
    g.N = ncols;
    g.K = lu->nlayr;
    g.AT = lu->LT + (int64_t)lu->pk * lu->nlayr * ld2;
    g.ldat = ld2;
    g.B = lu->U + (int64_t)lu->pk * lu->nlayr * ldu + u_col_off;
    g.ldb = ldu;
    g.C = lu->A11 + (int64_t)fnpr * lu->Nl + col_lo;
    g.ldc = lu->Nl;
    g.D = lu->A11 + (int64_t)fnpr * lu->Nl + col_lo;
    g.ldd = lu->Nl;
    g.alpha = -1.0;
    g.beta = 1.0;
    const int e = 4 * k + 2 * part;
    if (lu->time_gemm) CFLX_CUDA(cudaEventRecord(lu->ev[e], s));
    if (lu->use_ozaki) CFLX_TRY(launch_ozaki_gemm(&lu->oz, g.M, g.N, 0, u_col_off, g.D, g.ldd, max_ctas, s));
    else CFLX_TRY(launch_gemm_tn(g, s));
    if (lu->time_gemm) CFLX_CUDA(cudaEventRecord(lu->ev[e + 1], s));
    lu->ev_used[e / 2] = lu->time_gemm;
    lu->gemm_flops += 2.0 * g.M * (double)g.N * g.K;
    lu->launches++;
    return CFLX_OK;
}

int finish_step(cflx_lu* lu, int k, int& fnpr) {
    cudaStream_t s = lu->comm->stream;
    const int v = lu->v, Px = lu->Px, Py = lu->Py, Pz = lu->Pz, Ml = lu->Ml, Nl = lu->Nl;
    const int pi = lu->pi, pj = lu->pj, pk = lu->pk;
    const int loff = (k / Py) * v, pjk = k % Py, pik = k % Px;
    const bool on_col = (pj == pjk), on_row = (pi == pik), layer0 = (pk == 0);
    const int c0 = loff + (pj <= pjk ? v : 0);
    const int ncols = Nl - c0;
    const int fnpr_old = fnpr;
    const int n_old = Ml - fnpr_old;
    const int64_t ldk = std::max<int64_t>(2, round_up(n_old, 2));
    int nR = 0;
    while ((1 << nR) < Px) ++nR;
    double* A00 = lu->A00 + (size_t)(k & 1) * v * v;
    double* A00T = lu->A00T + (size_t)(k & 1) * v * v;
    {
        PhaseTimer t(lu, RG_step1_A00Buff_bcast, s);
        if (lu->P > 1) {
            const int root = (pik * Py + pjk) * Pz;
            if (lu->rank == root) {
                CFLX_TRY(launch_pack_bcast(A00, lu->tagsH, v, lu->bcast, s));
                lu->launches++;
            }
            CFLX_NCCL(ncclBroadcast(lu->bcast, lu->bcast, (size_t)v * v + v, ncclDouble, root, lu->comm->world, s));
            CFLX_TRY(launch_unpack_bcast(lu->bcast, v, A00, A00T, lu->gpivots, s));
            lu->launches++;
        } else {
            CFLX_CUDA(cudaMemcpyAsync(lu->gpivots, lu->tagsH, v * sizeof(int), cudaMemcpyDeviceToDevice, s));
        }
        CFLX_TRY(launch_record_pivots(lu->gpivots, v, lu->hist, k, s));
        lu->launches++;
    }
    {
        PhaseTimer t(lu, RG_step2_pushingpivots, s);
        CFLX_TRY(launch_plan_moves(lu->gpivots, v, Px, pi, fnpr_old, Ml, lu->igri, lu->plan, s));
        lu->launches++;
        if (Px > 1) {
            CFLX_CUDA(cudaMemcpyAsync(lu->h_npiv, lu->plan.npiv, sizeof(int), cudaMemcpyDeviceToHost, s));
            CFLX_CUDA(cudaEventRecord(lu->ev_npiv, s));
        }
        const int col_lo = layer0 ? 0 : loff;
        const int64_t ldu0 = std::max(2, ncols);
        CFLX_TRY(launch_push_phase1(lu->A11, Nl, Nl, col_lo, lu->plan, v, lu->tmp, ncols > 0 ? lu->A01raw : nullptr, ldu0, c0,
                                    s));
        CFLX_TRY(launch_push_phase2(lu->A11, Nl, Nl, col_lo, lu->plan, v, s));
        CFLX_TRY(launch_push_phase3(lu->A11, Nl, Nl, col_lo, fnpr_old, lu->plan, v, lu->tmp, s));
        CFLX_TRY(launch_update_gri(lu->gri, lu->gri_tmp, lu->igri, lu->plan.rowsrc, fnpr_old, Ml, v, Px, s));
        lu->launches += 5;
    }
    const int64_t ldu = std::max(2, ncols);
    const bool fused_l = (nR == 0);
    if (ncols > 0 && Px * Pz > 1) {
        PhaseTimer t(lu, RG_step2_reduce, s);
        CFLX_NCCL(ncclReduce(lu->A01raw, lu->A01raw, (size_t)v * ldu, ncclDouble, ncclSum, pik * Pz, lu->ik_comm.c, s));
    }
    if (layer0 && ((on_col && !fused_l) || on_row)) {
        PhaseTimer t(lu, RG_step5_dtrsm, s);
        CFLX_TRY(launch_diag_inverses(A00, v, lu->nb, lu->Uinv, lu->LinvT, s));
        lu->launches++;
    }
    const bool split_u = (lu->P == 1) && (k + 1 < lu->Nt) && ncols > v;
    const int ncols_a = split_u ? v : ncols;
    if (on_row && layer0 && ncols > 0) {
        PhaseTimer t(lu, RG_step5_dtrsm, s);
        CFLX_TRY(trsm_left_lower_unit(A00T, lu->LinvT, v, lu->nb, lu->A01raw, lu->U, ldu, ncols_a, s));
        lu->launches += 2 * (v / lu->nb) - 1;
    }
    if (Px * Pz > 1 && ncols > 0) {
        PhaseTimer t(lu, RG_step5_comm, s);
        CFLX_NCCL(ncclBroadcast(lu->U, lu->U, (size_t)v * ldu, ncclDouble, pik * Pz, lu->ik_comm.c, s));
    }
    auto store_factors = [&]() -> int {
        if (!layer0) return CFLX_OK;
        PhaseTimer t(lu, RG_storingresults, s);
        if (ncols > 0) {
            CFLX_TRY(launch_store_u_rows(lu->A11, Nl, fnpr_old, lu->plan, lu->U, ldu, c0, ncols, v, s));
            lu->launches++;
        }
        if (on_col) {
            CFLX_TRY(launch_store_diag(lu->A11, Nl, fnpr_old, lu->plan, A00, loff, v, s));
            lu->launches++;
        }
        return CFLX_OK;
    };
    if (!split_u) CFLX_TRY(store_factors());
    int npiv = v;
    if (Px > 1) {
        CFLX_CUDA(cudaEventSynchronize(lu->ev_npiv));
        npiv = *lu->h_npiv;
    }
    if (npiv < 0 || npiv > v || fnpr_old + npiv > Ml) {
        set_last_error("step %d: inconsistent pivot count %d (fnpr %d, Ml %d)", k, npiv, fnpr_old, Ml);
        return CFLX_ERR_STATE;
    }
    fnpr = fnpr_old + npiv;
    const int n_act = Ml - fnpr;
    const int64_t ld2 = std::max<int64_t>(2, round_up(n_act, 2));
    if (on_col && layer0 && n_act > 0) {
        {
            PhaseTimer t(lu, RG_step4_reshuffling, s);
            CFLX_TRY(launch_compact_panel(fused_l ? lu->W : lu->PT, ldk, fused_l ? lu->LT : lu->PT2, ld2, lu->plan.rowsrc,
                                          fnpr_old, lu->plan.npiv, Ml, v, s));
            lu->launches++;
        }
        if (!fused_l) {
            PhaseTimer t(lu, RG_step4_dtrsm, s);
            CFLX_TRY(trsm_right_upper_T(A00, lu->Uinv, v, lu->nb, lu->PT2, lu->LT, ld2, n_act, s));
            lu->launches += 2 * (v / lu->nb) - 1;
        }
        PhaseTimer t(lu, RG_storingresults, s);
        CFLX_TRY(launch_store_panel_T(lu->A11, Nl, fnpr, loff, n_act, v, lu->LT, ld2, s));
        lu->launches++;
    }
    if (Py * Pz > 1 && n_act > 0) {
        PhaseTimer t(lu, RG_step4_comm, s);
        CFLX_NCCL(ncclBroadcast(lu->LT, lu->LT, (size_t)v * ld2, ncclDouble, pjk * Pz, lu->jk_comm.c, s));
    }
    const bool next_col = (k + 1 < lu->Nt) && (pj == (k + 1) % Py);
    CFLX_TRY(ozaki_planes_a(lu, n_act, ld2, s));
    if (n_act > 0) CFLX_TRY(ozaki_planes_b(lu, 0, split_u ? std::min(v, ncols) : ncols, ldu, s));
    if (next_col) {
        const int w = std::min(v, ncols);
        CFLX_TRY(trailing_gemm(lu, k, 0, fnpr, n_act, c0, w, ld2, ldu, 0, s));
        cudaStream_t side = (lu->prof_mode == 1) ? nullptr : lu->side;
        cudaStream_t sp = side ? side : s;
        if (side) {
            CFLX_CUDA(cudaEventRecord(lu->ev_fork, s));
            CFLX_CUDA(cudaStreamWaitEvent(sp, lu->ev_fork, 0));
        }
        CFLX_TRY(panel_phase(lu, k + 1, fnpr, sp));
        if (side) CFLX_CUDA(cudaEventRecord(lu->ev_join, sp));
        if (split_u) {
            PhaseTimer t(lu, RG_step5_dtrsm, s);
            CFLX_TRY(trsm_left_lower_unit(A00T, lu->LinvT, v, lu->nb, lu->A01raw + v, lu->U + v, ldu, ncols - v, s));
            lu->launches += 2 * (v / lu->nb) - 1;
        }
        if (split_u) CFLX_TRY(store_factors());
        if (split_u && n_act > 0) CFLX_TRY(ozaki_planes_b(lu, w, ncols - w, ldu, s));
        const int leave = (side && lu->use_ozaki) ? lu->pws.cta_cap : 0;
        CFLX_TRY(trailing_gemm(lu, k, 1, fnpr, n_act, c0 + w, ncols - w, ld2, ldu, w, s, leave > 0 ? lu->oz.sms - leave : 0));
        if (side) CFLX_CUDA(cudaStreamWaitEvent(s, lu->ev_join, 0));
    } else {
        CFLX_TRY(trailing_gemm(lu, k, 0, fnpr, n_act, c0, ncols, ld2, ldu, 0, s));
    }
    return CFLX_OK;
}

void free_lu(cflx_lu* lu) {
    if (!lu) return;
    cudaSetDevice(lu->comm->device);
    double* dbl[] = {lu->PT, lu->PT2, lu->W, lu->LT, lu->A01raw, lu->U, lu->tmp, lu->A00, lu->A00T, lu->Uinv, lu->LinvT,
                     lu->candH, lu->S, lu->W2, lu->bcast, lu->Cbuf, lu->xbuf};
    for (double* p : dbl) cudaFree(p);
    int* ints[] = {lu->gri, lu->gri_tmp, lu->igri, lu->perm, lu->gpivots, lu->tagsH, lu->tagsS, lu->hist, lu->plan_mem,
                   lu->idx_buf};
    for (int* p : ints) cudaFree(p);
    if (lu->h_npiv) cudaFreeHost(lu->h_npiv);
    if (lu->pws.slot_hdr) panel_workspace_destroy(&lu->pws);
    for (auto& e : lu->ev) cudaEventDestroy(e);
    for (auto& e : lu->tl_pool) cudaEventDestroy(e);
    if (lu->ev_fork) cudaEventDestroy(lu->ev_fork);
    if (lu->ev_join) cudaEventDestroy(lu->ev_join);
    if (lu->ev_npiv) cudaEventDestroy(lu->ev_npiv);
    if (lu->copy) cudaStreamDestroy(lu->copy);
    if (lu->ev_a0_read) cudaEventDestroy(lu->ev_a0_read);
    if (lu->ev_upload) cudaEventDestroy(lu->ev_upload);
    for (SubComm* sc : {&lu->jk_comm, &lu->ik_comm})
        if (sc->c) ncclCommDestroy(sc->c);
    handle_free(lu);
    delete lu;
}

SolveFactor lu_solve_factor(cflx_lu* lu) { return SolveFactor{*lu, lu->Cbuf, lu->Ml, &lu->jk_comm, &lu->ik_comm, lu->Pz}; }

int lu_solve_prepare(cflx_lu* lu) {
    cudaStream_t s = lu->comm->stream;
    const int v = lu->v, Px = lu->Px, Ml = lu->Ml;
    std::vector<int> hist(lu->M);
    CFLX_TRY(cflx_lu_get_permutation(lu, hist.data()));
    if (lu->pk == 0) {
        cudaFree(lu->sv.inv);
        lu->sv.inv = nullptr;
        if (!lu->Cbuf) CFLX_TRY(dmalloc(&lu->Cbuf, (size_t)Ml * lu->Nl));
        int rc = redistribute_pivoted_rows(lu, hist, true, lu->A11, lu->Cbuf);
        cudaFree(lu->xbuf);
        lu->xbuf = nullptr;
        if (rc) return rc;
        CFLX_TRY(solve_inverses(&lu->sv, lu_solve_factor(lu), false));
        if (lu->pj == 0) {
            std::vector<int> rows(Ml, 0);
            for (int q = 0; q < lu->M; ++q) {
                const int k = q / v;
                if (k % Px == lu->pi) rows[(k / Px) * v + q % v] = hist[q];
            }
            CFLX_TRY(solve_set_rows(&lu->sv.rows, rows, s));
        }
    }
    lu->sv.ready = true;
    lu->sv.trans_ready = false;
    return CFLX_OK;
}

int lu_solve_prepare_trans(cflx_lu* lu) {
    cudaStream_t s = lu->comm->stream;
    const int v = lu->v, Px = lu->Px, Py = lu->Py;
    std::vector<int> hist(lu->M);
    CFLX_TRY(cflx_lu_get_permutation(lu, hist.data()));
    std::vector<int> unperm(lu->M);
    for (int q = 0; q < lu->M; ++q) unperm[hist[q]] = q;
    CFLX_TRY(solve_set_rows(&lu->sv.unperm, unperm, s));
    if (lu->pk == 0 && lu->pj == 0) {
        std::vector<int> rows(lu->Ml, 0);
        for (int q = 0; q < lu->M; ++q)
            if ((q / v) % Px == lu->pi) rows[(q / v / Px) * v + q % v] = q;
        CFLX_TRY(solve_set_rows(&lu->sv.rows_id, rows, s));
    }
    if (lu->pk == 0 && lu->pi == 0) {
        std::vector<int> cols(lu->Nl, 0);
        for (int q = 0; q < lu->M; ++q)
            if ((q / v) % Py == lu->pj) cols[(q / v / Py) * v + q % v] = q;
        CFLX_TRY(solve_set_rows(&lu->sv.cols, cols, s));
    }
    lu->sv.trans_ready = true;
    return CFLX_OK;
}

int lu_sweeps(cflx_lu* lu, bool transposed, bool pa, int nrhs, const double* B, int ldb, double* X, int ldx) {
    if (!lu->sv.ready) CFLX_TRY(lu_solve_prepare(lu));
    if ((transposed || pa) && !lu->sv.trans_ready) CFLX_TRY(lu_solve_prepare_trans(lu));
    const SolveFactor f = lu_solve_factor(lu);
    SolveCache* sc = &lu->sv;
    const int ldn = (int)round_up(nrhs, 8);
    CFLX_TRY(solve_cache_grow(sc, f, ldn, true, transposed, transposed));
    if (!transposed) {
        CFLX_TRY(solve_seed(sc, f, ldn, nrhs, B, ldb, SolveSeed{false, pa ? sc->rows_id : sc->rows, lu->Ml, sc->W}));
        CFLX_TRY(solve_row_sweep(sc, f, ldn, true, sc->W, lu->Px, true));
        CFLX_TRY(solve_row_sweep(sc, f, ldn, false, sc->X, 1, false));
        return solve_finish(sc, f, ldn, nrhs, X, ldx);
    }
    CFLX_TRY(solve_seed(sc, f, ldn, nrhs, B, ldb, SolveSeed{true, sc->cols, lu->Nl, sc->Z}));
    CFLX_TRY(solve_col_sweep(sc, f, ldn, true, Tri::UpperT, sc->Z, lu->Py, true));
    CFLX_TRY(solve_col_sweep(sc, f, ldn, false, Tri::UnitLowerT, sc->X, 1, false));
    return solve_finish(sc, f, ldn, nrhs, X, ldx, pa ? nullptr : sc->unperm);
}

const HandleTexts kLuTexts = {
    "%s requested before cflx_lu_factor, or after cflx_lu_set_local without a factorisation",
    "equilibration requested before cflx_lu_set_local",
    "equilibration refused: the input is already scaled (equed = '%c'); upload it again first"};

int lu_check(const cflx_lu* lu, const char* what, bool own_input) {
    CFLX_TRY(handle_check(lu, what));
    if (own_input && lu->a0_is_next) {
        set_last_error("%s refused: the input buffer of the last run was handed to the queued next matrix", what);
        return CFLX_ERR_STATE;
    }
    return CFLX_OK;
}

int lu_rcond(cflx_lu* lu, bool inf, double* rcond_out, double* anorm_out) {
    double anorm = 0.0, ainvnm = 0.0;
    CFLX_TRY(inf ? norminf_grid(*lu, lu->A0, &anorm) : norm1_grid(*lu, lu->A0, false, &anorm));
    if (anorm > 0.0) {
        auto apply = [&](int kase, double* x) { return lu_sweeps(lu, (kase == 2) != inf, true, 1, x, 1, x, 1); };
        CFLX_TRY(estimate_inv_norm1(lu->M, apply, &ainvnm));
    }
    *rcond_out = rcond_from(anorm, ainvnm);
    if (anorm_out) *anorm_out = anorm;
    return CFLX_OK;
}

RefineOp lu_refine_op(cflx_lu* lu, bool t) {
    auto solve = [lu, t](bool tk, int n, const double* b, int lb, double* x, int lx) {
        return lu_sweeps(lu, t != tk, false, n, b, lb, x, lx);
    };
    return RefineOp{*lu, lu->A0, t ? ResidMode::TN : ResidMode::NN, false, solve};
}
}

extern "C" {

const char* cflx_last_error(void) { return g_err; }
const char* cflx_version(void) { return "conflux_b200 0.1 (sm_90a)"; }

int cflx_device_count(int* count) {
    int n = 0;
    cudaError_t e = cudaGetDeviceCount(&n);
    if (e != cudaSuccess) {
        n = 0;
        cudaGetLastError();
    }
    *count = n;
    return CFLX_OK;
}

int cflx_get_unique_id(void* id_out) {
    static_assert(sizeof(ncclUniqueId) == CFLX_UNIQUE_ID_BYTES, "unique id size");
    ncclUniqueId id;
    CFLX_NCCL(ncclGetUniqueId(&id));
    std::memcpy(id_out, &id, sizeof(id));
    return CFLX_OK;
}

int cflx_comm_create(int world_size, int world_rank, const void* unique_id, int device, cflx_comm** out) {
    if (!out || world_size < 1 || world_rank < 0 || world_rank >= world_size) return CFLX_ERR_ARG;
    int ndev = 0;
    cflx_device_count(&ndev);
    if (ndev == 0) {
        set_last_error("no CUDA device visible: conflux_b200 has no CPU fallback");
        return CFLX_ERR_NO_DEVICE;
    }
    if (device < 0 || device >= ndev) {
        set_last_error("device %d out of range (%d visible)", device, ndev);
        return CFLX_ERR_ARG;
    }
    CFLX_CUDA(cudaSetDevice(device));
    auto* c = new cflx_comm;
    c->world_size = world_size;
    c->world_rank = world_rank;
    c->device = device;
    CFLX_CUDA(cudaStreamCreateWithFlags(&c->stream, cudaStreamNonBlocking));
    CFLX_CUDA(cudaMalloc((void**)&c->d_scratch, sizeof(double)));
    CFLX_CUDA(cudaMemset(c->d_scratch, 0, sizeof(double)));
    if (world_size > 1) {
        if (!unique_id) {
            set_last_error("unique_id required for world_size > 1");
            return CFLX_ERR_ARG;
        }
        ncclUniqueId id;
        std::memcpy(&id, unique_id, sizeof(id));
        CFLX_NCCL(ncclCommInitRank(&c->world, world_size, id, world_rank));
    }
    *out = c;
    return CFLX_OK;
}

int cflx_comm_barrier(cflx_comm* c) {
    if (!c) return CFLX_ERR_ARG;
    CFLX_CUDA(cudaSetDevice(c->device));
    return grid_barrier(c);
}

void cflx_comm_destroy(cflx_comm* c) {
    if (!c) return;
    cudaSetDevice(c->device);
    if (c->world) ncclCommDestroy(c->world);
    if (c->stream) cudaStreamDestroy(c->stream);
    cudaFree(c->d_scratch);
    delete c;
}

int cflx_auto_grid(int M, int N, int P, int* Px, int* Py, int* Pz) {
    if (M <= 0 || N <= 0 || P <= 0) return CFLX_ERR_ARG;
    const double ratio = 1.0 * std::max(M, N) / std::min(M, N);
    const int p1 = (int)std::cbrt(P / ratio);
    const int psq = (int)std::sqrt(P / ratio);
    const int phs = (int)std::sqrt(P / (2 * ratio));
    if (P == psq * psq) {
        *Px = psq; *Py = psq; *Pz = 1;
        return CFLX_OK;
    }
    if (phs * phs == P / 2) {
        *Px = phs; *Py = phs; *Pz = 2;
        return CFLX_OK;
    }
    int d[3] = {p1, (int)(ratio * p1), 0};
    d[2] = P / (d[0] * d[1]);
    std::sort(d, d + 3, [](int a, int b) { return a > b; });
    *Px = d[0]; *Py = d[1]; *Pz = d[2];
    return CFLX_OK;
}

int cflx_lu_dims(int M, int N, int v, int Px, int Py, int Pz, int* o) {
    if (M <= 0 || N <= 0 || v <= 0 || Px <= 0 || Py <= 0 || Pz <= 0 || !o) return CFLX_ERR_ARG;
    const int tx = (int)std::ceil((double)M / (v * Px)), ty = (int)std::ceil((double)N / (v * Py));
    const int Mp = v * Px * tx, Np = v * Py * ty;
    const int Nt = (int)std::ceil((double)Np / v), Mt = (int)std::ceil((double)Mp / v);
    o[0] = Mp; o[1] = Np;
    o[2] = (int)std::ceil((double)Mt / Px) * v;
    o[3] = (int)std::ceil((double)Nt / Py) * v;
    o[4] = Nt; o[5] = (v + Pz - 1) / Pz; o[6] = Mt; o[7] = Px * Py * Pz;
    return CFLX_OK;
}

int cflx_init_matrix_host(int M, int N, int v, int Px, int Py, int Pz, int rank, int seed, double* out) {
    int d[8];
    CFLX_TRY(cflx_lu_dims(M, N, v, Px, Py, Pz, d));
    const int Ml = d[2], Nl = d[3];
    if (rank < 0 || rank >= d[7] || !out) return CFLX_ERR_ARG;
    std::fill(out, out + (size_t)Ml * Nl, 0.0);
    if (rank % Pz != 0) return CFLX_OK;
    if (d[0] == d[1]) {
        std::vector<double> tab;
        if (fixed_input_matrix(d[0], &tab)) {
            const int n = d[0];
            const Layout L{n, v, d[4], Ml, Nl, Px, Py, rank / (Py * Pz), (rank / Pz) % Py};
            for (int lr = 0; lr < Ml; ++lr)
                for (int lc = 0; lc < Nl; ++lc) out[(size_t)lr * Nl + lc] = tab[(size_t)L.row(lr) * n + L.col(lc)];
            return CFLX_OK;
        }
    }
    std::mt19937_64 eng((unsigned long long)(seed + rank));
    std::uniform_real_distribution<double> dist;
    for (int lti = 0; lti < Ml / v; ++lti)
        for (int ltj = 0; ltj < Nl / v; ++ltj)
            for (int li = 0; li < v; ++li)
                for (int lj = 0; lj < v; ++lj) out[(size_t)(lti * v + li) * Nl + ltj * v + lj] = 5 + dist(eng);
    return CFLX_OK;
}

int cflx_lu_create(cflx_comm* c, int M, int N, int v, int Px, int Py, int Pz, cflx_lu** out) {
    if (!c || !out || M <= 0 || N <= 0 || v <= 0) return CFLX_ERR_ARG;
    CFLX_CUDA(cudaSetDevice(c->device));
    if (Px <= 0 || Py <= 0 || Pz <= 0) CFLX_TRY(cflx_auto_grid(M, N, c->world_size, &Px, &Py, &Pz));
    if (Px != Py) {
        set_last_error("grid %dx%dx%d: the CONFLUX LU path requires Px == Py (SURVEY.md fact 6)", Px, Py, Pz);
        return CFLX_ERR_UNSUPPORTED;
    }
    if (Px * Py * Pz != c->world_size) {
        set_last_error("grid %dx%dx%d does not match the %d ranks of the communicator", Px, Py, Pz, c->world_size);
        return CFLX_ERR_ARG;
    }
    if (v % 4 != 0 || v % Pz != 0 || (v / Pz) % 4 != 0 || pick_nb(v) == 0) {
        set_last_error("tile size v=%d unsupported: need v %% 4 == 0 and (v / Pz) %% 4 == 0", v);
        return CFLX_ERR_UNSUPPORTED;
    }
    int d[8];
    CFLX_TRY(cflx_lu_dims(M, N, v, Px, Py, Pz, d));
    if (d[0] != d[1]) {
        set_last_error("only square matrices are supported (the miniapp passes M = N)");
        return CFLX_ERR_UNSUPPORTED;
    }
    auto* lu = new cflx_lu;
    lu->M = d[0]; lu->N = d[1]; lu->Ml = d[2]; lu->Nl = d[3]; lu->Nt = d[4]; lu->nlayr = d[5]; lu->Mt = d[6];
    lu->v = v;
    lu->nb = pick_nb(v);
    int rc = CFLX_OK;
    auto fail = [&](int code) {
        free_lu(lu);
        return code;
// ... 408 lines not shown
```

conflux_b200/csrc/rows.cu:

```cuda
#include <algorithm>

#include "common.cuh"
#include "kernels.h"

namespace cflx {

namespace {

__global__ void extract_panel_T_kernel(const double* __restrict__ A, int64_t lda, int64_t row0, int64_t col0, int n,
                                       int v, double* __restrict__ PT, int64_t ldp) {
    __shared__ double tile[32][33];
    const int r0 = blockIdx.x * 32, c0 = blockIdx.y * 32;
    for (int dy = threadIdx.y; dy < 32; dy += blockDim.y) {
        const int r = r0 + dy, c = c0 + threadIdx.x;
        if (r < n && c < v) tile[dy][threadIdx.x] = A[(row0 + r) * lda + col0 + c];
    }
    __syncthreads();
    for (int dy = threadIdx.y; dy < 32; dy += blockDim.y) {
        const int c = c0 + dy, r = r0 + threadIdx.x;
        if (r < n && c < v) PT[(int64_t)c * ldp + r] = tile[threadIdx.x][dy];
    }
}
__global__ void store_panel_T_kernel(double* __restrict__ A, int64_t lda, int64_t row0, int64_t col0, int n, int v,
                                     const double* __restrict__ LT, int64_t ldp) {
    __shared__ double tile[32][33];
    const int r0 = blockIdx.x * 32, c0 = blockIdx.y * 32;
    for (int dy = threadIdx.y; dy < 32; dy += blockDim.y) {
        const int c = c0 + dy, r = r0 + threadIdx.x;
        if (r < n && c < v) tile[dy][threadIdx.x] = LT[(int64_t)c * ldp + r];
    }
    __syncthreads();
    for (int dy = threadIdx.y; dy < 32; dy += blockDim.y) {
        const int r = r0 + dy, c = c0 + threadIdx.x;
        if (r < n && c < v) A[(row0 + r) * lda + col0 + c] = tile[threadIdx.x][dy];
    }
}

__global__ void gather_winners_kernel(const double* __restrict__ PT, int64_t ldp, const int* __restrict__ tags,
                                      int n_valid, const int* __restrict__ perm, int v, double* __restrict__ out,
                                      int64_t ldo, int* __restrict__ out_tags, int dst0) {
    const int64_t e = (int64_t)blockIdx.x * blockDim.x + threadIdx.x;
    if (e >= (int64_t)v * v) return;
    const int c = (int)(e / v), i = (int)(e % v);
    const int src = perm[i];
    out[(int64_t)c * ldo + dst0 + i] = src < n_valid ? PT[(int64_t)c * ldp + src] : 0.0;
    if (c == 0) out_tags[dst0 + i] = src < n_valid ? tags[src] : 0;
}
__global__ void gather_a00_kernel(const double* __restrict__ W, int64_t ldw, const int* __restrict__ perm, int v, int nb,
                                  double* __restrict__ A00, double* __restrict__ A00T) {
    const int64_t e = (int64_t)blockIdx.x * blockDim.x + threadIdx.x;
    if (e >= (int64_t)v * v) return;
    const int i = (int)(e / v), c = (int)(e % v);
    double val;
    if (nb <= 0 || c < (i / nb) * nb) {
        val = W[(int64_t)c * ldw + perm[i]];
        A00[e] = val;
    } else {
        val = A00[e];
    }
    A00T[(int64_t)c * v + i] = val;
}

__global__ void __launch_bounds__(256) plan_moves_kernel(const int* __restrict__ gpivots, int v, int Px, int pi, int fnpr,
                                                         int Ml, const int* __restrict__ igri, MovePlan plan) {
    extern __shared__ int sm[];
    int* mine = sm;
    int* prow = sm + v;
    __shared__ int s_npiv, s_nel;
    const int t = threadIdx.x, T = blockDim.x;
    for (int i = t; i < v; i += T) mine[i] = ((gpivots[i] / v) % Px == pi) ? 1 : 0;
    for (int r = fnpr + t; r < Ml; r += T) plan.rowsrc[r] = r;
    __syncthreads();
    for (int i = t; i < v; i += T) {
        int rank = 0;
        for (int j = 0; j < i; ++j) rank += mine[j];
        if (mine[i]) {
            const int g = gpivots[i];
            const int lidx = (g / (v * Px)) * v + g % v;
            const int lrow = igri[lidx];
            plan.cur_piv[rank] = lrow;
            plan.order[rank] = i;
            plan.slot2piv[i] = rank;
            prow[rank] = lrow;
        } else {
            plan.slot2piv[i] = -1;
        }
        if (i == v - 1) s_npiv = rank + mine[i];
    }
    __syncthreads();
    const int npiv = s_npiv;
    for (int i = t; i < npiv; i += T) {
        const int r = fnpr + i;
        bool isp = false;
        for (int j = 0; j < npiv; ++j) isp = isp || (prow[j] == r);
        mine[i] = isp ? 0 : 1;
    }
    __syncthreads();
    for (int i = t; i < npiv; i += T) {
        if (mine[i]) {
            int rank = 0;
            for (int j = 0; j < i; ++j) rank += mine[j];
            plan.early[rank] = fnpr + i;
        }
        const int pr = prow[i];
        if (pr >= fnpr + npiv) {
            int rank = 0;
            for (int j = 0; j < npiv; ++j) rank += (prow[j] >= fnpr + npiv && prow[j] < pr) ? 1 : 0;
            plan.late[rank] = pr;
        }
    }
    if (t == 0) {
        int ne = 0;
        for (int j = 0; j < npiv; ++j) ne += mine[j];
        s_nel = ne;
        plan.npiv[0] = npiv;
        plan.nel[0] = ne;
    }
    __syncthreads();
    const int nel = s_nel;
    for (int i = t; i < nel; i += T) plan.rowsrc[plan.late[i]] = plan.early[i];
    for (int i = t; i < npiv; i += T) plan.rowsrc[fnpr + i] = prow[i];
}

__device__ __forceinline__ void copy_row_seg(double* __restrict__ dst, const double* __restrict__ src, int len, int chunk,
                                             int nchunks) {
    const int n2 = len >> 1;
    const int per = (n2 + nchunks - 1) / nchunks;
    const int b = chunk * per, e = min(n2, b + per);
    const double2* s2 = reinterpret_cast<const double2*>(src);
    double2* d2 = reinterpret_cast<double2*>(dst);
    for (int i = b + threadIdx.x; i < e; i += blockDim.x) d2[i] = s2[i];
}
__global__ void push_phase1_kernel(const double* __restrict__ A, int64_t lda, int ncols, int col_lo, MovePlan plan, int v,
                                   double* __restrict__ tmp, double* __restrict__ a01raw, int64_t ld01, int c0) {
    const int npiv = plan.npiv[0];
    const int y = blockIdx.y;
    if (y < v) {
        if (y >= npiv) return;
        const int src = plan.cur_piv[y];
        copy_row_seg(tmp + (int64_t)y * lda + col_lo, A + (int64_t)src * lda + col_lo, ncols - col_lo, blockIdx.x,
                     gridDim.x);
    } else if (a01raw != nullptr) {
        const int slot = y - v;
        const int p = plan.slot2piv[slot];
        const int len = ncols - c0;
        double* dst = a01raw + (int64_t)slot * ld01;
        if (p >= 0) {
            copy_row_seg(dst, A + (int64_t)plan.cur_piv[p] * lda + c0, len, blockIdx.x, gridDim.x);
        } else {
            const int n2 = len >> 1;
            const int per = (n2 + gridDim.x - 1) / gridDim.x;
            const int b = blockIdx.x * per, e = min(n2, b + per);
            double2* d2 = reinterpret_cast<double2*>(dst);
            for (int i = b + threadIdx.x; i < e; i += blockDim.x) d2[i] = make_double2(0.0, 0.0);
        }
    }
}
__global__ void push_phase2_kernel(double* __restrict__ A, int64_t lda, int ncols, int col_lo, MovePlan plan) {
    if ((int)blockIdx.y >= plan.nel[0]) return;
    const int src = plan.early[blockIdx.y], dst = plan.late[blockIdx.y];
    copy_row_seg(A + (int64_t)dst * lda + col_lo, A + (int64_t)src * lda + col_lo, ncols - col_lo, blockIdx.x, gridDim.x);
}
__global__ void push_phase3_kernel(double* __restrict__ A, int64_t lda, int ncols, int col_lo, int fnpr, MovePlan plan,
                                   const double* __restrict__ tmp) {
    if ((int)blockIdx.y >= plan.npiv[0]) return;
    copy_row_seg(A + (int64_t)(fnpr + blockIdx.y) * lda + col_lo, tmp + (int64_t)blockIdx.y * lda + col_lo, ncols - col_lo,
                 blockIdx.x, gridDim.x);
}

__global__ void gri_gather_kernel(const int* __restrict__ gri, int* __restrict__ gri_tmp, const int* __restrict__ rowsrc,
                                  int fnpr, int Ml) {
    const int r = fnpr + blockIdx.x * blockDim.x + threadIdx.x;
    if (r < Ml) gri_tmp[r] = gri[rowsrc[r]];
}
__global__ void gri_commit_kernel(int* __restrict__ gri, const int* __restrict__ gri_tmp, int* __restrict__ igri, int fnpr,
                                  int Ml, int v, int Px) {
    const int r = fnpr + blockIdx.x * blockDim.x + threadIdx.x;
    if (r < Ml) {
        const int g = gri_tmp[r];
        gri[r] = g;
        igri[(g / (v * Px)) * v + g % v] = r;
    }
}
__global__ void compact_panel_kernel(const double* __restrict__ PT, int64_t ldp, double* __restrict__ PT2, int64_t ldp2,
                                     const int* __restrict__ rowsrc, int fnpr_old, const int* __restrict__ npiv, int Ml) {
    const int fnpr_new = fnpr_old + npiv[0];
    const int rp = blockIdx.x * blockDim.x + threadIdx.x;
    const int c = blockIdx.y;
    if (fnpr_new + rp < Ml) PT2[(int64_t)c * ldp2 + rp] = PT[(int64_t)c * ldp + (rowsrc[fnpr_new + rp] - fnpr_old)];
}
__global__ void store_u_rows_kernel(double* __restrict__ A, int64_t lda, int fnpr_old, MovePlan plan,
                                    const double* __restrict__ U, int64_t ldu, int c0, int ncols) {
    if ((int)blockIdx.y >= plan.npiv[0]) return;
    const int i = blockIdx.y;
    copy_row_seg(A + (int64_t)(fnpr_old + i) * lda + c0, U + (int64_t)plan.order[i] * ldu, ncols, blockIdx.x, gridDim.x);
}
__global__ void store_diag_kernel(double* __restrict__ A, int64_t lda, int fnpr_old, MovePlan plan,
                                  const double* __restrict__ A00, int loff, int v) {
    if ((int)blockIdx.y >= plan.npiv[0]) return;
    const int i = blockIdx.y;
    const double* src = A00 + (int64_t)plan.order[i] * v;
    double* dst = A + (int64_t)(fnpr_old + i) * lda + loff;
    for (int c = threadIdx.x; c < v; c += blockDim.x) dst[c] = src[c];
}

__global__ void fill_kernel(double* p, int64_t n, double val) {
    const int64_t i = (int64_t)blockIdx.x * blockDim.x + threadIdx.x;
    if (i < n) p[i] = val;
}
__global__ void iota_gri_kernel(int* gri, int* igri, int Ml, int v, int Px, int pi) {
    const int i = blockIdx.x * blockDim.x + threadIdx.x;
    if (i < Ml) {
        gri[i] = (i % v) + ((i / v) * Px + pi) * v;
        igri[i] = i;
    }
}
__global__ void pack_bcast_kernel(const double* A00, const int* tags, int v, double* buf) {
    const int i = blockIdx.x * blockDim.x + threadIdx.x;
    if (i < v * v) buf[i] = A00[i];
    if (i < v) buf[v * v + i] = (double)tags[i];
}
__global__ void unpack_bcast_kernel(const double* buf, int v, double* A00, double* A00T, int* gpivots) {
    const int e = blockIdx.x * blockDim.x + threadIdx.x;
    if (e < v * v) {
        const int i = e / v, c = e % v;
        const double x = buf[e];
        A00[e] = x;
        A00T[c * v + i] = x;
    }
    if (e < v) gpivots[e] = (int)buf[v * v + e];
}
__global__ void record_pivots_kernel(const int* gpivots, int v, int* hist, int k) {
    const int i = blockIdx.x * blockDim.x + threadIdx.x;
    if (i < v) hist[(int64_t)k * v + i] = gpivots[i];
}

__global__ void split_factors_kernel(const double* __restrict__ F, int64_t ldf, int n, double* __restrict__ LT,
                                     double* __restrict__ U) {
    __shared__ double tile[32][33];
    const int r0 = blockIdx.y * 32, c0 = blockIdx.x * 32;
    for (int dy = threadIdx.y; dy < 32; dy += blockDim.y) {
        const int r = r0 + dy, c = c0 + threadIdx.x;
        double x = 0.0;
        if (r < n && c < n) x = F[(int64_t)r * ldf + c];
        tile[dy][threadIdx.x] = x;
        if (r < n && c < n) U[(int64_t)r * n + c] = (c >= r) ? x : 0.0;
    }
    __syncthreads();
    for (int dy = threadIdx.y; dy < 32; dy += blockDim.y) {
        const int k = c0 + dy, m = r0 + threadIdx.x;
        if (k < n && m < n) LT[(int64_t)k * n + m] = (m > k) ? tile[threadIdx.x][dy] : (m == k ? 1.0 : 0.0);
    }
}
__global__ void gather_perm_rows_kernel(const double* __restrict__ A, int64_t lda, const int* __restrict__ perm, int n,
                                        double* __restrict__ out) {
    const int r = blockIdx.x;
    const double* src = A + (int64_t)perm[r] * lda;
    double* dst = out + (int64_t)r * n;
    for (int c = blockIdx.y * blockDim.x + threadIdx.x; c < n; c += gridDim.y * blockDim.x) dst[c] = src[c];
}
__device__ __forceinline__ double block_sum(double s) {
    for (int o = 16; o > 0; o >>= 1) s += __shfl_xor_sync(0xffffffffu, s, o);
    __shared__ double w[32];
    if ((threadIdx.x & 31) == 0) w[threadIdx.x >> 5] = s;
    __syncthreads();
    if (threadIdx.x < 32) {
        s = threadIdx.x < (blockDim.x >> 5) ? w[threadIdx.x] : 0.0;
        for (int o = 16; o > 0; o >>= 1) s += __shfl_xor_sync(0xffffffffu, s, o);
    }
    return s;
}
__global__ void sumsq_partial_kernel(const double* __restrict__ X, int64_t count, double* __restrict__ partials) {
    double s = 0.0;
    for (int64_t i = (int64_t)blockIdx.x * blockDim.x + threadIdx.x; i < count; i += (int64_t)gridDim.x * blockDim.x)
        s = fma(X[i], X[i], s);
    s = block_sum(s);
    if (threadIdx.x == 0) partials[blockIdx.x] = s;
}
__global__ void sumsq_final_kernel(const double* __restrict__ partials, int n, double* __restrict__ out) {
    double s = 0.0;
    for (int i = threadIdx.x; i < n; i += blockDim.x) s += partials[i];
    s = block_sum(s);
    if (threadIdx.x == 0) *out += s;
}

inline int row_chunks(int len) {
    int c = (len / 2 + 2047) / 2048;
    return c < 1 ? 1 : (c > 64 ? 64 : c);
}
}

#define POST_LAUNCH()                     \
    do {                                  \
        CFLX_CUDA(cudaGetLastError());    \
        return CFLX_OK;                   \
    } while (0)

int launch_extract_panel_T(const double* A, int64_t lda, int64_t row0, int64_t col0, int n, int v, double* PT,
                           int64_t ldp, cudaStream_t s) {
    if (n <= 0) return CFLX_OK;
    dim3 grid((n + 31) / 32, (v + 31) / 32), block(32, 8);
    extract_panel_T_kernel<<<grid, block, 0, s>>>(A, lda, row0, col0, n, v, PT, ldp);
    POST_LAUNCH();
}
int launch_store_panel_T(double* A, int64_t lda, int64_t row0, int64_t col0, int n, int v, const double* LT, int64_t ldp,
                         cudaStream_t s) {
    if (n <= 0) return CFLX_OK;
    dim3 grid((n + 31) / 32, (v + 31) / 32), block(32, 8);
    store_panel_T_kernel<<<grid, block, 0, s>>>(A, lda, row0, col0, n, v, LT, ldp);
    POST_LAUNCH();
}
int launch_gather_winners(const double* PT, int64_t ldp, const int* tags, int n_valid, const int* perm, int v,
                          double* out_vals, int64_t ldo, int* out_tags, int dst0, cudaStream_t s) {
    const int64_t tot = (int64_t)v * v;
    gather_winners_kernel<<<(unsigned)((tot + 255) / 256), 256, 0, s>>>(PT, ldp, tags, n_valid, perm, v, out_vals, ldo,
                                                                        out_tags, dst0);
    POST_LAUNCH();
}
int launch_gather_a00(const double* W, int64_t ldw, const int* perm, int v, int nb, double* A00, double* A00T,
                      cudaStream_t s) {
    const int64_t tot = (int64_t)v * v;
    gather_a00_kernel<<<(unsigned)((tot + 255) / 256), 256, 0, s>>>(W, ldw, perm, v, nb, A00, A00T);
    POST_LAUNCH();
}
int launch_plan_moves(const int* gpivots, int v, int Px, int pi, int fnpr, int Ml, const int* igri, MovePlan plan,
                      cudaStream_t s) {
    plan_moves_kernel<<<1, 256, 2 * v * sizeof(int), s>>>(gpivots, v, Px, pi, fnpr, Ml, igri, plan);
    POST_LAUNCH();
}
int launch_push_phase1(const double* A, int64_t lda, int ncols, int col_lo, MovePlan plan, int v, double* tmp,
                       double* a01raw, int64_t ld01, int c0, cudaStream_t s) {
    dim3 grid(row_chunks(ncols), a01raw ? 2 * v : v);
    push_phase1_kernel<<<grid, 256, 0, s>>>(A, lda, ncols, col_lo, plan, v, tmp, a01raw, ld01, c0);
    POST_LAUNCH();
}
int launch_push_phase2(double* A, int64_t lda, int ncols, int col_lo, MovePlan plan, int v, cudaStream_t s) {
    dim3 grid(row_chunks(ncols), v);
    push_phase2_kernel<<<grid, 256, 0, s>>>(A, lda, ncols, col_lo, plan);
    POST_LAUNCH();
}
int launch_push_phase3(double* A, int64_t lda, int ncols, int col_lo, int fnpr, MovePlan plan, int v, const double* tmp,
                       cudaStream_t s) {
    dim3 grid(row_chunks(ncols), v);
    push_phase3_kernel<<<grid, 256, 0, s>>>(A, lda, ncols, col_lo, fnpr, plan, tmp);
    POST_LAUNCH();
}
int launch_update_gri(int* gri, int* gri_tmp, int* igri, const int* rowsrc, int fnpr, int Ml, int v, int Px,
                      cudaStream_t s) {
    const int n = Ml - fnpr;
    if (n <= 0) return CFLX_OK;
    gri_gather_kernel<<<(n + 255) / 256, 256, 0, s>>>(gri, gri_tmp, rowsrc, fnpr, Ml);
    gri_commit_kernel<<<(n + 255) / 256, 256, 0, s>>>(gri, gri_tmp, igri, fnpr, Ml, v, Px);
    POST_LAUNCH();
}
int launch_compact_panel(const double* PT, int64_t ldp, double* PT2, int64_t ldp2, const int* rowsrc, int fnpr_old,
                         const int* npiv, int Ml, int v, cudaStream_t s) {
    const int n = Ml - fnpr_old;
    if (n <= 0) return CFLX_OK;
    dim3 grid((n + 255) / 256, v);
    compact_panel_kernel<<<grid, 256, 0, s>>>(PT, ldp, PT2, ldp2, rowsrc, fnpr_old, npiv, Ml);
    POST_LAUNCH();
}
int launch_store_u_rows(double* A, int64_t lda, int fnpr_old, MovePlan plan, const double* U, int64_t ldu, int c0,
                        int ncols, int v, cudaStream_t s) {
    if (ncols <= 0) return CFLX_OK;
    dim3 grid(row_chunks(ncols), v);
    store_u_rows_kernel<<<grid, 256, 0, s>>>(A, lda, fnpr_old, plan, U, ldu, c0, ncols);
    POST_LAUNCH();
}
int launch_store_diag(double* A, int64_t lda, int fnpr_old, MovePlan plan, const double* A00, int loff, int v,
                      cudaStream_t s) {
    dim3 grid(1, v);
    store_diag_kernel<<<grid, 128, 0, s>>>(A, lda, fnpr_old, plan, A00, loff, v);
    POST_LAUNCH();
}
int launch_split_factors(const double* F, int64_t ldf, int n, double* LT, double* U, cudaStream_t s) {
    dim3 grid((n + 31) / 32, (n + 31) / 32), block(32, 8);
    split_factors_kernel<<<grid, block, 0, s>>>(F, ldf, n, LT, U);
    POST_LAUNCH();
}
int launch_gather_perm_rows(const double* A, int64_t lda, const int* perm, int n, double* out, cudaStream_t s) {
    dim3 grid(n, std::max(1, std::min(32, n / 256)));
    gather_perm_rows_kernel<<<grid, 256, 0, s>>>(A, lda, perm, n, out);
    POST_LAUNCH();
}
int launch_sumsq(const double* X, int64_t count, double* out, double* partials, cudaStream_t s) {
    sumsq_partial_kernel<<<SUMSQ_PARTIALS, 256, 0, s>>>(X, count, partials);
    CFLX_CUDA(cudaGetLastError());
    return launch_sum_partials(partials, SUMSQ_PARTIALS, out, s);
}
int launch_sum_partials(const double* partials, int n, double* out, cudaStream_t s) {
    sumsq_final_kernel<<<1, 1024, 0, s>>>(partials, n, out);
    POST_LAUNCH();
}
int launch_fill(double* p, int64_t n, double val, cudaStream_t s) {
    if (n <= 0) return CFLX_OK;
    fill_kernel<<<(unsigned)((n + 255) / 256), 256, 0, s>>>(p, n, val);
    POST_LAUNCH();
}
int launch_iota_gri(int* gri, int* igri, int Ml, int v, int Px, int pi, cudaStream_t s) {
    iota_gri_kernel<<<(Ml + 255) / 256, 256, 0, s>>>(gri, igri, Ml, v, Px, pi);
    POST_LAUNCH();
}
int launch_pack_bcast(const double* A00, const int* tags, int v, double* buf, cudaStream_t s) {
    pack_bcast_kernel<<<(v * v + 255) / 256, 256, 0, s>>>(A00, tags, v, buf);
    POST_LAUNCH();
}
int launch_unpack_bcast(const double* buf, int v, double* A00, double* A00T, int* gpivots, cudaStream_t s) {
    unpack_bcast_kernel<<<(v * v + 255) / 256, 256, 0, s>>>(buf, v, A00, A00T, gpivots);
    POST_LAUNCH();
}
int launch_record_pivots(const int* gpivots, int v, int* hist, int k, cudaStream_t s) {
    record_pivots_kernel<<<(v + 255) / 256, 256, 0, s>>>(gpivots, v, hist, k);
    POST_LAUNCH();
}

}
```

conflux_b200/csrc/trsm.cu:

```cuda
#include "common.cuh"
#include "kernels.h"

namespace cflx {
namespace {
template <int NB>
__global__ void __launch_bounds__(1024) diag_inverse_kernel(const double* __restrict__ A00, int v, double* __restrict__ Uinv,
                                                            double* __restrict__ LinvT) {
    constexpr int EPL = (NB + 31) / 32;
    extern __shared__ double S[];
    constexpr int LD = NB + 1;
    const int j = blockIdx.x;
    const int warp = threadIdx.x >> 5, lane = threadIdx.x & 31, nwarps = blockDim.x >> 5;
    const double* blk = A00 + (size_t)(j * NB) * v + j * NB;
    for (int e = threadIdx.x; e < NB * NB; e += blockDim.x) S[(e / NB) * LD + e % NB] = blk[(size_t)(e / NB) * v + e % NB];
    __syncthreads();
    double* out = (blockIdx.y == 0 ? Uinv : LinvT) + (size_t)j * NB * NB;
    const int cols_per = (NB + gridDim.z - 1) / gridDim.z;
    const int c_lo = blockIdx.z * cols_per, c_hi = min(NB, c_lo + cols_per);
    for (int c = c_lo + warp; c < c_hi; c += nwarps) {
        double x[EPL];
#pragma unroll
        for (int e = 0; e < EPL; ++e) x[e] = 0.0;
        if (blockIdx.y == 0) {
            const double xc = 1.0 / S[c * LD + c];
#pragma unroll
            for (int e = 0; e < EPL; ++e)
                if (lane + 32 * e == c) x[e] = xc;
            for (int r = c - 1; r >= 0; --r) {
                double s = 0.0;
#pragma unroll
                for (int e = 0; e < EPL; ++e) {
                    const int t = lane + 32 * e;
                    if (t > r && t <= c) s = fma(S[r * LD + t], x[e], s);
                }
#pragma unroll
                for (int o = 16; o > 0; o >>= 1) s += __shfl_xor_sync(0xffffffffu, s, o);
                const double xr = -s / S[r * LD + r];
#pragma unroll
                for (int e = 0; e < EPL; ++e)
                    if (lane + 32 * e == r) x[e] = xr;
            }
#pragma unroll
            for (int e = 0; e < EPL; ++e) {
                const int t = lane + 32 * e;
                if (t < NB) out[(size_t)t * NB + c] = x[e];
            }
        } else {
#pragma unroll
            for (int e = 0; e < EPL; ++e)
                if (lane + 32 * e == c) x[e] = 1.0;
            for (int r = c + 1; r < NB; ++r) {
                double s = 0.0;
#pragma unroll
                for (int e = 0; e < EPL; ++e) {
                    const int t = lane + 32 * e;
                    if (t >= c && t < r) s = fma(S[r * LD + t], x[e], s);
                }
#pragma unroll
                for (int o = 16; o > 0; o >>= 1) s += __shfl_xor_sync(0xffffffffu, s, o);
#pragma unroll
                for (int e = 0; e < EPL; ++e)
                    if (lane + 32 * e == r) x[e] = -s;
            }
#pragma unroll
            for (int e = 0; e < EPL; ++e) {
                const int t = lane + 32 * e;
                if (t < NB) out[(size_t)c * NB + t] = x[e];
            }
        }
    }
}

template <int NB>
int launch_diag_nb(const double* A00, int v, double* Uinv, double* LinvT, cudaStream_t stream) {
    constexpr size_t smem = (size_t)NB * (NB + 1) * sizeof(double);
    constexpr int CS = NB > 64 ? NB / 32 : 1;
    const int warps = NB < 32 ? NB : 32;
    static PerDeviceMax cfg;
    if (cfg.raise(smem))
        CFLX_CUDA(cudaFuncSetAttribute(diag_inverse_kernel<NB>, cudaFuncAttributeMaxDynamicSharedMemorySize, (int)smem));
    diag_inverse_kernel<NB><<<dim3(v / NB, 2, CS), 32 * warps, smem, stream>>>(A00, v, Uinv, LinvT);
    CFLX_CUDA(cudaGetLastError());
    return CFLX_OK;
}
}

int launch_diag_inverses(const double* A00, int v, int nb, double* Uinv, double* LinvT, cudaStream_t stream) {
    switch (nb) {
        case 128: return launch_diag_nb<128>(A00, v, Uinv, LinvT, stream);
        case 64: return launch_diag_nb<64>(A00, v, Uinv, LinvT, stream);
        case 32: return launch_diag_nb<32>(A00, v, Uinv, LinvT, stream);
        case 16: return launch_diag_nb<16>(A00, v, Uinv, LinvT, stream);
        case 8: return launch_diag_nb<8>(A00, v, Uinv, LinvT, stream);
        case 4: return launch_diag_nb<4>(A00, v, Uinv, LinvT, stream);
        default:
            set_last_error("diag_inverses: unsupported block size %d", nb);
            return CFLX_ERR_UNSUPPORTED;
    }
}

int trsm_right_upper_T(const double* A00, const double* Uinv, int v, int nb, double* PT, double* LT, int64_t ld, int n,
                       cudaStream_t stream) {
    if (n <= 0) return CFLX_OK;
    const int nblk = v / nb;
    const int N = (n + 1) & ~1;
    for (int j = 0; j < nblk; ++j) {
        GemmArgs g{};
        g.M = nb; g.N = N; g.K = nb;
        g.AT = Uinv + (size_t)j * nb * nb; g.ldat = nb;
        g.B = PT + (int64_t)j * nb * ld; g.ldb = ld;
        g.C = nullptr; g.ldc = ld;
        g.D = LT + (int64_t)j * nb * ld; g.ldd = ld;
        g.alpha = 1.0; g.beta = 0.0;
        CFLX_TRY(launch_gemm_tn(g, stream));
        const int rest = v - (j + 1) * nb;
        if (rest > 0) {
            GemmArgs u{};
            u.M = rest; u.N = N; u.K = nb;
            u.AT = A00 + (size_t)(j * nb) * v + (j + 1) * nb; u.ldat = v;
            u.B = LT + (int64_t)j * nb * ld; u.ldb = ld;
            u.C = PT + (int64_t)(j + 1) * nb * ld; u.ldc = ld;
            u.D = PT + (int64_t)(j + 1) * nb * ld; u.ldd = ld;
            u.alpha = -1.0; u.beta = 1.0;
            CFLX_TRY(launch_gemm_tn(u, stream));
        }
    }
    return CFLX_OK;
}

int trsm_left_lower_unit(const double* A00T, const double* LinvT, int v, int nb, double* R, double* U, int64_t ld, int n,
                         cudaStream_t stream) {
    if (n <= 0) return CFLX_OK;
    const int nblk = v / nb;
    for (int j = 0; j < nblk; ++j) {
        GemmArgs g{};
        g.M = nb; g.N = n; g.K = nb;
        g.AT = LinvT + (size_t)j * nb * nb; g.ldat = nb;
        g.B = R + (int64_t)j * nb * ld; g.ldb = ld;
        g.C = nullptr; g.ldc = ld;
        g.D = U + (int64_t)j * nb * ld; g.ldd = ld;
        g.alpha = 1.0; g.beta = 0.0;
        CFLX_TRY(launch_gemm_tn(g, stream));
        const int rest = v - (j + 1) * nb;
        if (rest > 0) {
            GemmArgs u{};
            u.M = rest; u.N = n; u.K = nb;
            u.AT = A00T + (size_t)(j * nb) * v + (j + 1) * nb; u.ldat = v;
            u.B = U + (int64_t)j * nb * ld; u.ldb = ld;
            u.C = R + (int64_t)(j + 1) * nb * ld; u.ldc = ld;
            u.D = R + (int64_t)(j + 1) * nb * ld; u.ldd = ld;
            u.alpha = -1.0; u.beta = 1.0;
            CFLX_TRY(launch_gemm_tn(u, stream));
        }
    }
    return CFLX_OK;
}

}
```

include/conflux_b200.h:

```cpp
#ifndef CONFLUX_B200_H
#define CONFLUX_B200_H

#include <stddef.h>
#include <stdint.h>

#ifdef __cplusplus
extern "C" {
#endif

typedef enum {
    CFLX_OK = 0,
    CFLX_ERR_ARG = -1,
    CFLX_ERR_CUDA = -2,
    CFLX_ERR_NCCL = -3,
    CFLX_ERR_UNSUPPORTED = -4,
    CFLX_ERR_STATE = -5,
    CFLX_ERR_NO_DEVICE = -6
} cflx_status;

typedef struct cflx_comm cflx_comm;
typedef struct cflx_lu cflx_lu;

#define CFLX_UNIQUE_ID_BYTES 128

const char* cflx_last_error(void);
const char* cflx_version(void);
int cflx_device_count(int* count);

int cflx_get_unique_id(void* id_out );
int cflx_comm_create(int world_size, int world_rank, const void* unique_id, int device, cflx_comm** out);
int cflx_comm_barrier(cflx_comm*);
void cflx_comm_destroy(cflx_comm*);

int cflx_host_alloc(size_t bytes, void** out);
int cflx_host_free(void* p);

int cflx_auto_grid(int M, int N, int P, int* Px, int* Py, int* Pz);
int cflx_lu_dims(int M, int N, int v, int Px, int Py, int Pz, int* dims_out);
int cflx_init_matrix_host(int M, int N, int v, int Px, int Py, int Pz, int rank, int seed, double* local_out);

int cflx_lu_create(cflx_comm*, int M, int N, int v, int Px, int Py, int Pz, cflx_lu** out);
int cflx_lu_info(const cflx_lu*, int* info_out);
int cflx_lu_set_local(cflx_lu*, const double* host_local);
int cflx_lu_queue_next_local(cflx_lu*, const double* host_next);
int cflx_lu_factor(cflx_lu*, double* ms_out);
int cflx_lu_get_factors(cflx_lu*, double* C_host, int* permutation_out);
int cflx_lu_get_permutation(cflx_lu*, int* permutation_out);
int cflx_lu_validate(cflx_lu*, double* frob_abs_out, double* frob_rel_out);
int cflx_lu_residual(cflx_lu*, double* rel_out);
int cflx_lu_solve(cflx_lu*, int nrhs, const double* B, int ldb, double* X, int ldx);
int cflx_lu_solve_trans(cflx_lu*, int nrhs, const double* B, int ldb, double* X, int ldx);
int cflx_lu_rcond(cflx_lu*, double* rcond_out, double* anorm_out);
int cflx_lu_refine(cflx_lu*, int trans, int nrhs, const double* B, int ldb, double* X, int ldx, double* ferr_out,
                   double* berr_out);
int cflx_lu_equilibrate(cflx_lu*, int apply, double* r_out, double* c_out, double* rowcnd_out, double* colcnd_out,
                        double* amax_out, char* equed_out, int* info_out);
int cflx_lu_svx(cflx_lu*, int trans, int nrhs, const double* B, int ldb, double* X, int ldx, double* rcond_out,
                double* ferr_out, double* berr_out, double* rpvgrw_out, char* equed_out, int* info_out);
int cflx_lu_inverse(cflx_lu*, double* Ainv_local, int* info_out);
int cflx_lu_det(cflx_lu*, int unscaled, double* sign_out, double* logabsdet_out, double* mant_out, int64_t* exp_out,
                int* info_out);
int cflx_lu_uses_ozaki(const cflx_lu*);
int cflx_lu_launch_count(cflx_lu*, int64_t* count_out, int reset);
int cflx_lu_set_profiling(cflx_lu*, int mode);
int cflx_lu_phase_ms(cflx_lu*, double* ms_out);
int cflx_lu_timeline(cflx_lu*, char* buf, int buf_len);
int cflx_lu_set_kernel_timing(cflx_lu*, int enabled);
int cflx_lu_trailing_stats(cflx_lu*, double* ms_out, double* flops_out);
void cflx_lu_destroy(cflx_lu*);

typedef struct cflx_chol cflx_chol;
int cflx_chol_auto_grid(int P, int N, int* grid3_out);
int cflx_chol_auto_tile(int N, int P, int Pz);
int cflx_chol_dims(int N, int v, int Px, int Py, int Pz, int* dims_out);
int cflx_chol_init_matrix_host(int N, int v, int Px, int Py, int Pz, int rank, double* local_out);
int cflx_chol_create(cflx_comm*, int N, int v, int Px, int Py, int Pz, cflx_chol** out);
int cflx_chol_info(const cflx_chol*, int* info_out);
int cflx_chol_set_local(cflx_chol*, const double* host_local);
int cflx_chol_factor(cflx_chol*, double* ms_out);
int cflx_chol_get_local(cflx_chol*, double* L_host);
int cflx_chol_validate(cflx_chol*, double* frob_abs_out, double* frob_rel_out);
int cflx_chol_solve(cflx_chol*, int nrhs, const double* B, int ldb, double* X, int ldx);
int cflx_chol_rcond(cflx_chol*, double* rcond_out, double* anorm_out);
int cflx_chol_refine(cflx_chol*, int nrhs, const double* B, int ldb, double* X, int ldx, double* ferr_out,
                     double* berr_out);
int cflx_chol_equilibrate(cflx_chol*, int apply, double* s_out, double* scond_out, double* amax_out, char* equed_out,
                          int* info_out);
int cflx_chol_svx(cflx_chol*, int nrhs, const double* B, int ldb, double* X, int ldx, double* rcond_out, double* ferr_out,
                  double* berr_out, char* equed_out, int* info_out);
int cflx_chol_inverse(cflx_chol*, double* Ainv_local);
int cflx_chol_det(cflx_chol*, int unscaled, double* logdet_out, double* mant_out, int64_t* exp_out);
int cflx_chol_launch_count(cflx_chol*, int64_t* count_out, int reset);
void cflx_chol_destroy(cflx_chol*);

int cflx_dbg_gemm_tn(int M, int N, int K, const double* AT, int at_rows, int64_t ldat, int64_t at_off, const double* B,
                     int b_rows, int64_t ldb, int64_t b_off, const double* C, int c_rows, int64_t ldc, int row_off,
                     int col_off, double alpha, double beta, int in_place, double* D_out, double* C_out, int reps,
                     double* ms_out);
int cflx_dbg_gemm_narrow(int M, int N, int K, const double* A, const double* B, const double* C, double alpha, double beta,
                         double* D, int reps, double* ms_out);
int cflx_dbg_gemm_narrow_tn(int M, int N, int K, const double* AT, const double* B, const double* C, double alpha,
                            double beta, double* D, int reps, double* ms_out);
int cflx_dbg_residual(int mode, int Ml, int Nl, const double* A, int v, int Kappa, int Px, int Py, int pi, int pj,
                      int nrhs, const double* Xc, const double* Xr, double* P_out, double* Q_out, int reps, double* ms_out);
int cflx_dbg_equil(int Ml, int Nl, int v, int Kappa, int Px, int Py, int pi, int pj, int M, const double* A,
                   const double* r, const double* c, char equed, int ncols, double* rowmax_out, double* colmax_out,
                   double* diag_out, double* scaled_out, double* sym_scaled_out, double* growth_out, int* zero_pivot_out);
int cflx_dbg_inverse_share(int mode, int Ml, int Nl, int v, int Kappa, int Px, int Py, int pi, int pj, int M, int c0,
                           int nc, int rows, const double* X, int ldx, const int* perm, double* W_out,
                           double* share_inout, int zero_fill);
int cflx_dbg_det(int n, const double* d, const double* s1, const double* s2, int square, double* mant_out,
                 int64_t* exp_out, int* neg_out, int* first_zero_out, int* nonfinite_out);
int cflx_dbg_panel(int n, int v, const double* panel, int* perm_out, double* A00_out, double* LU_out, int reps,
                   double* ms_out);
int cflx_dbg_trsm(int n, int v, int nb, int64_t ld, const double* A00, const double* B, double* X_out, const double* R,
                  double* Y_out);
int cflx_dbg_diag_inverse(int v, int nb, const double* A00, double* Uinv_out, double* LinvT_out);
int cflx_dbg_potrf_tile(int v, const double* A, double* L_out, double* LT_out, int* info_out, int variant);
int cflx_dbg_ozaki_gemm(int M, int N, int K, int row0, int col0, int max_ctas, const double* AT, const double* B,
                        const double* C, double* D, signed char* planesA_out, signed char* planesB_out, int* ea_out,
                        int* eb_out, int reps, double* ms_out, double* split_ms_out);
int cflx_dbg_wgmma_peak(int n, double* tmacs_out);
int cflx_dbg_push_pivots(int n_rows, int n_cols, double* A_inout, int npiv, const int* pivot_rows, int fnpr, int* gri_out,
                         double* a01_out);
int cflx_dbg_fp64_peak(int which, double* tflops_out);
int cflx_dbg_fp64_peak_ex(int which, double* burst_out, double* sustained_out);

#ifdef __cplusplus
}
#endif
#endif
```

Before: 25210.

## Split pivot push around lookahead panel, overlap diag inverses, auto-pick GEMM tile

On a single GPU, the row-swap push is split in two. First only the next panel's column window is swapped, so the lookahead panel can start early. The remaining columns are swapped after the panel is launched, overlapping with it. Diagonal-block inverses move to the side stream, and several redundant copies are removed: the panel copy into W, the gpivots copy, and the gather of the candidate values. GEMM now chooses the 64 tile automatically when the 128-tile grid would leave most SMs idle. The extra code paths add complexity and more kernel launches, and they risk ordering bugs between streams.

New measurement: 26490 (median of 6 runs). 1.05x the previous value.

```diff
diff --git a/conflux_b200/__init__.py b/conflux_b200/__init__.py
--- a/conflux_b200/__init__.py
+++ b/conflux_b200/__init__.py
@@ -602,6 +602,15 @@
         return A, gri, a01[:len(piv)]
 
     @staticmethod
+    def push_split(A, pivot_rows, fnpr, loff, c0, w):
+        A = np.array(A, dtype=np.float64, order="C")
+        piv = np.ascontiguousarray(pivot_rows, dtype=np.int32)
+        a01 = np.zeros((len(piv), A.shape[1] - c0))
+        check(lib().cflx_dbg_push_split(A.shape[0], A.shape[1], A.ctypes.data, len(piv), piv.ctypes.data, int(fnpr), int(loff),
+                                        int(c0), int(w), a01.ctypes.data), "dbg_push_split")
+        return A, a01
+
+    @staticmethod
     def wgmma_peak(n):
         t = ctypes.c_double()
         check(lib().cflx_dbg_wgmma_peak(int(n), ctypes.byref(t)), "dbg_wgmma_peak")
diff --git a/conflux_b200/_lib.py b/conflux_b200/_lib.py
--- a/conflux_b200/_lib.py
+++ b/conflux_b200/_lib.py
@@ -20,7 +20,7 @@
     "cflx_lu_get_permutation", "cflx_lu_residual", "cflx_lu_validate", "cflx_lu_solve", "cflx_lu_solve_trans", "cflx_lu_rcond", "cflx_lu_refine", "cflx_lu_equilibrate", "cflx_lu_svx", "cflx_lu_inverse", "cflx_lu_det", "cflx_lu_launch_count", "cflx_lu_uses_ozaki", "cflx_lu_set_profiling", "cflx_lu_phase_ms", "cflx_lu_timeline",
     "cflx_lu_set_kernel_timing", "cflx_lu_trailing_stats", "cflx_lu_destroy", "cflx_chol_auto_grid", "cflx_chol_auto_tile", "cflx_chol_dims", "cflx_chol_init_matrix_host",
     "cflx_chol_create", "cflx_chol_info", "cflx_chol_set_local", "cflx_chol_factor", "cflx_chol_get_local", "cflx_chol_validate",
-    "cflx_chol_solve", "cflx_chol_rcond", "cflx_chol_refine", "cflx_chol_equilibrate", "cflx_chol_svx", "cflx_chol_inverse", "cflx_chol_det", "cflx_chol_launch_count", "cflx_chol_destroy", "cflx_dbg_gemm_tn", "cflx_dbg_gemm_narrow", "cflx_dbg_gemm_narrow_tn", "cflx_dbg_residual", "cflx_dbg_equil", "cflx_dbg_inverse_share", "cflx_dbg_det", "cflx_dbg_panel", "cflx_dbg_trsm", "cflx_dbg_diag_inverse", "cflx_dbg_potrf_tile", "cflx_dbg_push_pivots", "cflx_dbg_ozaki_gemm", "cflx_dbg_wgmma_peak", "cflx_dbg_fp64_peak", "cflx_dbg_fp64_peak_ex",
+    "cflx_chol_solve", "cflx_chol_rcond", "cflx_chol_refine", "cflx_chol_equilibrate", "cflx_chol_svx", "cflx_chol_inverse", "cflx_chol_det", "cflx_chol_launch_count", "cflx_chol_destroy", "cflx_dbg_gemm_tn", "cflx_dbg_gemm_narrow", "cflx_dbg_gemm_narrow_tn", "cflx_dbg_residual", "cflx_dbg_equil", "cflx_dbg_inverse_share", "cflx_dbg_det", "cflx_dbg_panel", "cflx_dbg_trsm", "cflx_dbg_diag_inverse", "cflx_dbg_potrf_tile", "cflx_dbg_push_pivots", "cflx_dbg_push_split", "cflx_dbg_ozaki_gemm", "cflx_dbg_wgmma_peak", "cflx_dbg_fp64_peak", "cflx_dbg_fp64_peak_ex",
 ]
 
 
@@ -128,6 +128,8 @@
         L.cflx_dbg_potrf_tile.argtypes = [ctypes.c_int] + [ctypes.c_void_p] * 4 + [ctypes.c_int]
         L.cflx_dbg_push_pivots.argtypes = [ctypes.c_int, ctypes.c_int, ctypes.c_void_p, ctypes.c_int, ctypes.c_void_p, ctypes.c_int,
                                            ctypes.c_void_p, ctypes.c_void_p]
+        L.cflx_dbg_push_split.argtypes = [ctypes.c_int, ctypes.c_int, ctypes.c_void_p, ctypes.c_int, ctypes.c_void_p] + [ctypes.c_int] * 4 + [
+            ctypes.c_void_p]
         L.cflx_dbg_ozaki_gemm.argtypes = [ctypes.c_int] * 6 + [ctypes.c_void_p] * 8 + [ctypes.c_int, c_double_p, c_double_p]
         L.cflx_dbg_wgmma_peak.argtypes = [ctypes.c_int, c_double_p]
         L.cflx_dbg_fp64_peak.argtypes = [ctypes.c_int, c_double_p]
diff --git a/conflux_b200/csrc/dbg.cu b/conflux_b200/csrc/dbg.cu
--- a/conflux_b200/csrc/dbg.cu
+++ b/conflux_b200/csrc/dbg.cu
@@ -580,6 +580,47 @@
     CFLX_CUDA(cudaMemcpy(A_inout, dA.p, 8 * (size_t)n_rows * n_cols, cudaMemcpyDeviceToHost));
     if (gri_out) CFLX_CUDA(cudaMemcpy(gri_out, dgri.p, sizeof(int) * n_rows, cudaMemcpyDeviceToHost));
     if (a01_out) CFLX_CUDA(cudaMemcpy(a01_out, da01.p, 8 * (size_t)v * n_cols, cudaMemcpyDeviceToHost));
+    CFLX_CUDA(cudaDeviceSynchronize());
+    return CFLX_OK;
+}
+
+int cflx_dbg_push_split(int n_rows, int n_cols, double* A_inout, int npiv, const int* pivot_rows, int fnpr, int loff,
+                        int c0, int w, double* a01_out) {
+    CFLX_TRY(check_device());
+    if (n_rows <= 0 || n_cols <= 0 || npiv <= 0 || npiv > n_rows - fnpr || fnpr < 0 || ((n_cols | loff | c0 | w) & 1) ||
+        loff < 0 || c0 < loff || w <= 0 || c0 + w > n_cols)
+        return CFLX_ERR_ARG;
+    const int v = npiv;
+    const int64_t ld01 = n_cols - c0;
+    DevBuf dA, dtmp, da01, dplan, dgp, digri;
+    CFLX_TRY(dA.alloc(8 * (size_t)n_rows * n_cols));
+    CFLX_TRY(dtmp.alloc(8 * (size_t)v * n_cols));
+    CFLX_TRY(da01.alloc(8 * (size_t)v * ld01));
+    CFLX_TRY(dplan.alloc(sizeof(int) * (6 * (size_t)v + 8 + n_rows)));
+    CFLX_TRY(dgp.alloc(sizeof(int) * v));
+    CFLX_TRY(digri.alloc(sizeof(int) * 2 * n_rows));
+    CFLX_CUDA(cudaMemcpy(dA.p, A_inout, 8 * (size_t)n_rows * n_cols, cudaMemcpyHostToDevice));
+    CFLX_CUDA(cudaMemcpy(dgp.p, pivot_rows, sizeof(int) * v, cudaMemcpyHostToDevice));
+    CFLX_CUDA(cudaMemset(da01.p, 0, 8 * (size_t)v * ld01));
+    MovePlan plan{};
+    int* pm = dplan.as<int>();
+    plan.npiv = pm; plan.nel = pm + 4; pm += 8;
+    plan.cur_piv = pm; pm += v;
+    plan.order = pm; pm += v;
+    plan.slot2piv = pm; pm += v;
+    plan.early = pm; pm += v;
+    plan.late = pm; pm += 2 * v;
+    plan.rowsrc = pm;
+    int* gri = digri.as<int>() + n_rows;
+    CFLX_TRY(launch_iota_gri(gri, digri.as<int>(), n_rows, n_rows, 1, 0, 0));
+    CFLX_TRY(launch_plan_moves(dgp.as<int>(), v, 1, 0, fnpr, n_rows, digri.as<int>(), plan, 0));
+    double* A = dA.as<double>();
+    CFLX_TRY(launch_push_window(A, n_cols, plan, v, da01.as<double>(), ld01, c0, w, 0));
+    CFLX_TRY(launch_push_phase1(A, n_cols, n_cols, 0, plan, v, dtmp.as<double>(), da01.as<double>() + w, ld01, c0 + w, 0,
+                                loff));
+    CFLX_TRY(launch_push_rest(A, n_cols, plan, fnpr, dtmp.as<double>(), loff, c0 + w, n_cols, 0));
+    CFLX_CUDA(cudaMemcpy(A_inout, dA.p, 8 * (size_t)n_rows * n_cols, cudaMemcpyDeviceToHost));
+    if (a01_out) CFLX_CUDA(cudaMemcpy(a01_out, da01.p, 8 * (size_t)v * ld01, cudaMemcpyDeviceToHost));
     CFLX_CUDA(cudaDeviceSynchronize());
     return CFLX_OK;
 }
diff --git a/conflux_b200/csrc/gemm.cu b/conflux_b200/csrc/gemm.cu
--- a/conflux_b200/csrc/gemm.cu
+++ b/conflux_b200/csrc/gemm.cu
@@ -204,9 +204,18 @@
     static int v = -1;
     if (v < 0) {
         const char* e = getenv("CFLX_GEMM_TILE");
-        v = (e && atoi(e) == 64) ? 64 : 128;
+        v = e ? atoi(e) : 0;
+        if (v != 64 && v != 128) v = 0;
     }
     return v;
+}
+int sm_count() {
+    static int n[64] = {};
+    int dev = 0;
+    cudaGetDevice(&dev);
+    if (dev < 0 || dev >= 64) return 0;
+    if (!n[dev]) cudaDeviceGetAttribute(&n[dev], cudaDevAttrMultiProcessorCount, dev);
+    return n[dev];
 }
 }
 
@@ -223,7 +232,12 @@
                        (long long)g.ldat, (long long)g.ldb, (long long)g.ldc, (long long)g.ldd);
         return CFLX_ERR_UNSUPPORTED;
     }
-    if (tile_variant() == 64) return launch_one<1, 4, 2>(g, stream);
+    int t = tile_variant();
+    if (!t) {
+        const int64_t ctas = (int64_t)((g.N + 127) / 128) * ((g.M + 127) / 128);
+        t = (g.fill_sms && 2 * ctas <= sm_count()) ? 64 : 128;
+    }
+    if (t == 64) return launch_one<1, 4, 2>(g, stream);
     return launch_one<2, 4, 1>(g, stream);
 }
 
diff --git a/conflux_b200/csrc/kernels.h b/conflux_b200/csrc/kernels.h
--- a/conflux_b200/csrc/kernels.h
+++ b/conflux_b200/csrc/kernels.h
@@ -16,6 +16,7 @@
     double* D;
     int64_t ldd;
     double alpha, beta;
+    bool fill_sms;
 };
 int gemm_tn_setup();
 int launch_gemm_tn(const GemmArgs& g, cudaStream_t stream);
@@ -76,10 +77,14 @@
 int launch_plan_moves(const int* gpivots, int v, int Px, int pi, int fnpr, int Ml, const int* igri, MovePlan plan,
                       cudaStream_t stream);
 int launch_push_phase1(const double* A, int64_t lda, int ncols, int col_lo, MovePlan plan, int v, double* tmp,
-                       double* a01raw, int64_t ld01, int c0, cudaStream_t stream);
+                       double* a01raw, int64_t ld01, int c0, cudaStream_t stream, int tmp_hi = -1);
 int launch_push_phase2(double* A, int64_t lda, int ncols, int col_lo, MovePlan plan, int v, cudaStream_t stream);
 int launch_push_phase3(double* A, int64_t lda, int ncols, int col_lo, int fnpr, MovePlan plan, int v,
                        const double* tmp, cudaStream_t stream);
+int launch_push_window(double* A, int64_t lda, MovePlan plan, int v, double* a01raw, int64_t ld01, int c0, int w,
+                       cudaStream_t stream);
+int launch_push_rest(double* A, int64_t lda, MovePlan plan, int fnpr, const double* tmp, int l_hi, int r_lo, int r_hi,
+                     cudaStream_t stream);
 int launch_update_gri(int* gri, int* gri_tmp, int* igri, const int* rowsrc, int fnpr, int Ml, int v, int Px,
                       cudaStream_t stream);
 int launch_compact_panel(const double* PT, int64_t ldp, double* PT2, int64_t ldp2, const int* rowsrc, int fnpr_old,
diff --git a/conflux_b200/csrc/lu.cu b/conflux_b200/csrc/lu.cu
--- a/conflux_b200/csrc/lu.cu
+++ b/conflux_b200/csrc/lu.cu
@@ -277,9 +277,10 @@
     const int64_t ldk = std::max<int64_t>(2, round_up(n_old, 2));
     int nR = 0;
     while ((1 << nR) < Px) ++nR;
+    const bool one = (lu->P == 1);
     {
         PhaseTimer t(lu, RG_step0_copy, s);
-        CFLX_TRY(launch_extract_panel_T(lu->A11, Nl, fnpr, loff, n_old, v, lu->PT, ldk, s));
+        CFLX_TRY(launch_extract_panel_T(lu->A11, Nl, fnpr, loff, n_old, v, one ? lu->W : lu->PT, ldk, s));
         lu->launches++;
     }
     if (Pz > 1 && n_old > 0) {
@@ -288,7 +289,7 @@
     }
     if (pk != 0) return CFLX_OK;
     int my_half = 0;
-    {
+    if (!one) {
         PhaseTimer t(lu, RG_step1_A10copy, s);
         CFLX_CUDA(cudaMemcpyAsync(lu->W, lu->PT, (size_t)v * ldk * sizeof(double), cudaMemcpyDeviceToDevice, s));
     }
@@ -310,7 +311,7 @@
         if (first_partner > Px - 1) first_partner = Px - 1;
         my_half = first_partner < pi ? 1 : 0;
         CFLX_TRY(launch_gather_winners(lu->PT, ldk, lu->gri + fnpr, n_old, lu->perm, v,
-                                       lu->candH + (size_t)my_half * v * v, v, lu->tagsH + my_half * v, 0, s));
+                                       one ? nullptr : lu->candH + (size_t)my_half * v * v, v, lu->tagsH + my_half * v, 0, s));
         lu->launches++;
     }
     PhaseTimer t(lu, RG_step1_pivoting, s);
@@ -368,6 +369,7 @@
     g.ldd = lu->Nl;
     g.alpha = -1.0;
     g.beta = 1.0;
+    g.fill_sms = (part == 0);
     const int e = 4 * k + 2 * part;
     if (lu->time_gemm) CFLX_CUDA(cudaEventRecord(lu->ev[e], s));
     if (lu->use_ozaki) CFLX_TRY(launch_ozaki_gemm(&lu->oz, g.M, g.N, 0, u_col_off, g.D, g.ldd, max_ctas, s));
@@ -394,6 +396,19 @@
     while ((1 << nR) < Px) ++nR;
     double* A00 = lu->A00 + (size_t)(k & 1) * v * v;
     double* A00T = lu->A00T + (size_t)(k & 1) * v * v;
+    const bool split_u = (lu->P == 1) && (k + 1 < lu->Nt) && ncols > v;
+    cudaStream_t inv_s = (lu->P == 1 && lu->prof_mode != 1) ? lu->side : nullptr;
+    if (inv_s) {
+        CFLX_CUDA(cudaEventRecord(lu->ev_fork, s));
+        CFLX_CUDA(cudaStreamWaitEvent(inv_s, lu->ev_fork, 0));
+        {
+            PhaseTimer t(lu, RG_step5_dtrsm, inv_s);
+            CFLX_TRY(launch_diag_inverses(A00, v, lu->nb, lu->Uinv, lu->LinvT, inv_s));
+            lu->launches++;
+        }
+        CFLX_CUDA(cudaEventRecord(lu->ev_join, inv_s));
+    }
+    const int* gpivots = lu->P > 1 ? lu->gpivots : lu->tagsH;
     {
         PhaseTimer t(lu, RG_step1_A00Buff_bcast, s);
         if (lu->P > 1) {
@@ -405,15 +420,13 @@
             CFLX_NCCL(ncclBroadcast(lu->bcast, lu->bcast, (size_t)v * v + v, ncclDouble, root, lu->comm->world, s));
             CFLX_TRY(launch_unpack_bcast(lu->bcast, v, A00, A00T, lu->gpivots, s));
             lu->launches++;
-        } else {
-            CFLX_CUDA(cudaMemcpyAsync(lu->gpivots, lu->tagsH, v * sizeof(int), cudaMemcpyDeviceToDevice, s));
-        }
-        CFLX_TRY(launch_record_pivots(lu->gpivots, v, lu->hist, k, s));
+        }
+        CFLX_TRY(launch_record_pivots(gpivots, v, lu->hist, k, s));
         lu->launches++;
     }
     {
         PhaseTimer t(lu, RG_step2_pushingpivots, s);
-        CFLX_TRY(launch_plan_moves(lu->gpivots, v, Px, pi, fnpr_old, Ml, lu->igri, lu->plan, s));
+        CFLX_TRY(launch_plan_moves(gpivots, v, Px, pi, fnpr_old, Ml, lu->igri, lu->plan, s));
         lu->launches++;
         if (Px > 1) {
             CFLX_CUDA(cudaMemcpyAsync(lu->h_npiv, lu->plan.npiv, sizeof(int), cudaMemcpyDeviceToHost, s));
@@ -421,12 +434,18 @@
         }
         const int col_lo = layer0 ? 0 : loff;
         const int64_t ldu0 = std::max(2, ncols);
-        CFLX_TRY(launch_push_phase1(lu->A11, Nl, Nl, col_lo, lu->plan, v, lu->tmp, ncols > 0 ? lu->A01raw : nullptr, ldu0, c0,
-                                    s));
-        CFLX_TRY(launch_push_phase2(lu->A11, Nl, Nl, col_lo, lu->plan, v, s));
-        CFLX_TRY(launch_push_phase3(lu->A11, Nl, Nl, col_lo, fnpr_old, lu->plan, v, lu->tmp, s));
+        if (split_u) {
+            CFLX_TRY(launch_push_window(lu->A11, Nl, lu->plan, v, lu->A01raw, ldu0, c0, v, s));
+            lu->launches++;
+        } else {
+            CFLX_TRY(launch_push_phase1(lu->A11, Nl, Nl, col_lo, lu->plan, v, lu->tmp, ncols > 0 ? lu->A01raw : nullptr, ldu0,
+                                        c0, s));
+            CFLX_TRY(launch_push_phase2(lu->A11, Nl, Nl, col_lo, lu->plan, v, s));
+            CFLX_TRY(launch_push_phase3(lu->A11, Nl, Nl, col_lo, fnpr_old, lu->plan, v, lu->tmp, s));
+            lu->launches += 3;
+        }
         CFLX_TRY(launch_update_gri(lu->gri, lu->gri_tmp, lu->igri, lu->plan.rowsrc, fnpr_old, Ml, v, Px, s));
-        lu->launches += 5;
+        lu->launches += 2;
     }
     const int64_t ldu = std::max(2, ncols);
     const bool fused_l = (nR == 0);
@@ -434,12 +453,13 @@
         PhaseTimer t(lu, RG_step2_reduce, s);
         CFLX_NCCL(ncclReduce(lu->A01raw, lu->A01raw, (size_t)v * ldu, ncclDouble, ncclSum, pik * Pz, lu->ik_comm.c, s));
     }
-    if (layer0 && ((on_col && !fused_l) || on_row)) {
+    if (inv_s) {
+        CFLX_CUDA(cudaStreamWaitEvent(s, lu->ev_join, 0));
+    } else if (layer0 && ((on_col && !fused_l) || on_row)) {
         PhaseTimer t(lu, RG_step5_dtrsm, s);
         CFLX_TRY(launch_diag_inverses(A00, v, lu->nb, lu->Uinv, lu->LinvT, s));
         lu->launches++;
     }
-    const bool split_u = (lu->P == 1) && (k + 1 < lu->Nt) && ncols > v;
     const int ncols_a = split_u ? v : ncols;
     if (on_row && layer0 && ncols > 0) {
         PhaseTimer t(lu, RG_step5_dtrsm, s);
@@ -488,10 +508,15 @@
             CFLX_TRY(trsm_right_upper_T(A00, lu->Uinv, v, lu->nb, lu->PT2, lu->LT, ld2, n_act, s));
             lu->launches += 2 * (v / lu->nb) - 1;
         }
+    }
+    auto store_l = [&]() -> int {
+        if (!(on_col && layer0 && n_act > 0)) return CFLX_OK;
         PhaseTimer t(lu, RG_storingresults, s);
         CFLX_TRY(launch_store_panel_T(lu->A11, Nl, fnpr, loff, n_act, v, lu->LT, ld2, s));
         lu->launches++;
-    }
+        return CFLX_OK;
+    };
+    if (!split_u) CFLX_TRY(store_l());
     if (Py * Pz > 1 && n_act > 0) {
         PhaseTimer t(lu, RG_step4_comm, s);
         CFLX_NCCL(ncclBroadcast(lu->LT, lu->LT, (size_t)v * ld2, ncclDouble, pjk * Pz, lu->jk_comm.c, s));
@@ -511,11 +536,18 @@
         CFLX_TRY(panel_phase(lu, k + 1, fnpr, sp));
         if (side) CFLX_CUDA(cudaEventRecord(lu->ev_join, sp));
         if (split_u) {
+            PhaseTimer t(lu, RG_step2_pushingpivots, s);
+            CFLX_TRY(launch_push_phase1(lu->A11, Nl, Nl, 0, lu->plan, v, lu->tmp, lu->A01raw + v, ldu, c0 + v, s, loff));
+            CFLX_TRY(launch_push_rest(lu->A11, Nl, lu->plan, fnpr_old, lu->tmp, loff, c0 + v, Nl, s));
+            lu->launches += 2;
+        }
+        if (split_u) {
             PhaseTimer t(lu, RG_step5_dtrsm, s);
             CFLX_TRY(trsm_left_lower_unit(A00T, lu->LinvT, v, lu->nb, lu->A01raw + v, lu->U + v, ldu, ncols - v, s));
             lu->launches += 2 * (v / lu->nb) - 1;
         }
         if (split_u) CFLX_TRY(store_factors());
+        if (split_u) CFLX_TRY(store_l());
         if (split_u && n_act > 0) CFLX_TRY(ozaki_planes_b(lu, w, ncols - w, ldu, s));
         const int leave = (side && lu->use_ozaki) ? lu->pws.cta_cap : 0;
         CFLX_TRY(trailing_gemm(lu, k, 1, fnpr, n_act, c0 + w, ncols - w, ld2, ldu, w, s, leave > 0 ? lu->oz.sms - leave : 0));
diff --git a/conflux_b200/csrc/rows.cu b/conflux_b200/csrc/rows.cu
--- a/conflux_b200/csrc/rows.cu
+++ b/conflux_b200/csrc/rows.cu
@@ -40,10 +40,10 @@
                                       int n_valid, const int* __restrict__ perm, int v, double* __restrict__ out,
                                       int64_t ldo, int* __restrict__ out_tags, int dst0) {
     const int64_t e = (int64_t)blockIdx.x * blockDim.x + threadIdx.x;
-    if (e >= (int64_t)v * v) return;
+    if (e >= (out ? (int64_t)v * v : v)) return;
     const int c = (int)(e / v), i = (int)(e % v);
     const int src = perm[i];
-    out[(int64_t)c * ldo + dst0 + i] = src < n_valid ? PT[(int64_t)c * ldp + src] : 0.0;
+    if (out) out[(int64_t)c * ldo + dst0 + i] = src < n_valid ? PT[(int64_t)c * ldp + src] : 0.0;
     if (c == 0) out_tags[dst0 + i] = src < n_valid ? tags[src] : 0;
 }
 __global__ void gather_a00_kernel(const double* __restrict__ W, int64_t ldw, const int* __restrict__ perm, int v, int nb,
@@ -131,14 +131,14 @@
     double2* d2 = reinterpret_cast<double2*>(dst);
     for (int i = b + threadIdx.x; i < e; i += blockDim.x) d2[i] = s2[i];
 }
-__global__ void push_phase1_kernel(const double* __restrict__ A, int64_t lda, int ncols, int col_lo, MovePlan plan, int v,
-                                   double* __restrict__ tmp, double* __restrict__ a01raw, int64_t ld01, int c0) {
+__global__ void push_phase1_kernel(const double* __restrict__ A, int64_t lda, int ncols, int col_lo, int tmp_hi, MovePlan plan,
+                                   int v, double* __restrict__ tmp, double* __restrict__ a01raw, int64_t ld01, int c0) {
     const int npiv = plan.npiv[0];
     const int y = blockIdx.y;
     if (y < v) {
         if (y >= npiv) return;
         const int src = plan.cur_piv[y];
-        copy_row_seg(tmp + (int64_t)y * lda + col_lo, A + (int64_t)src * lda + col_lo, ncols - col_lo, blockIdx.x,
+        copy_row_seg(tmp + (int64_t)y * lda + col_lo, A + (int64_t)src * lda + col_lo, tmp_hi - col_lo, blockIdx.x,
                      gridDim.x);
     } else if (a01raw != nullptr) {
         const int slot = y - v;
@@ -168,6 +168,57 @@
                  blockIdx.x, gridDim.x);
 }
 
+template <class Src, class Dst>
+__device__ __forceinline__ void move_chunk_rows(int n, int lanes, int w2, Src src, Dst dst) {
+    const int lane = threadIdx.x % lanes, R = blockDim.x / lanes;
+    if (lane >= w2) return;
+    for (int i = threadIdx.x / lanes; i < n; i += 4 * R) {
+        double2 x[4];
+#pragma unroll
+        for (int u = 0; u < 4; ++u)
+            if (i + u * R < n) x[u] = src(i + u * R, lane);
+#pragma unroll
+        for (int u = 0; u < 4; ++u)
+            if (i + u * R < n) dst(i + u * R)[lane] = x[u];
+    }
+}
+__global__ void push_window_kernel(double* A, int64_t lda, MovePlan plan, int v, double* __restrict__ a01raw, int64_t ld01,
+                                   int c0, int w, int lanes) {
+    const int b2 = blockIdx.x * lanes, w2 = min(lanes, w / 2 - b2);
+    double2* A2 = reinterpret_cast<double2*>(A + c0) + b2;
+    const int64_t lda2 = lda / 2;
+    double2* o2 = reinterpret_cast<double2*>(a01raw) + b2;
+    move_chunk_rows(
+        v, lanes, w2,
+        [&](int i, int l) {
+            const int p = plan.slot2piv[i];
+            return p >= 0 ? A2[(int64_t)plan.cur_piv[p] * lda2 + l] : make_double2(0.0, 0.0);
+        },
+        [&](int i) { return o2 + (int64_t)i * (ld01 / 2); });
+    __syncthreads();
+    move_chunk_rows(
+        plan.nel[0], lanes, w2, [&](int i, int l) { return A2[(int64_t)plan.early[i] * lda2 + l]; },
+        [&](int i) { return A2 + (int64_t)plan.late[i] * lda2; });
+}
+__global__ void push_rest_kernel(double* A, int64_t lda, MovePlan plan, int fnpr, const double* __restrict__ tmp, int l_hi,
+                                 int r_lo, int r_hi, int lanes) {
+    const int nl = (l_hi / 2 + lanes - 1) / lanes;
+    const bool left = (int)blockIdx.x < nl;
+    const int b2 = left ? blockIdx.x * lanes : r_lo / 2 + (blockIdx.x - nl) * lanes;
+    const int w2 = min(lanes, (left ? l_hi : r_hi) / 2 - b2);
+    double2* A2 = reinterpret_cast<double2*>(A) + b2;
+    const int64_t lda2 = lda / 2;
+    move_chunk_rows(
+        plan.nel[0], lanes, w2, [&](int i, int l) { return A2[(int64_t)plan.early[i] * lda2 + l]; },
+        [&](int i) { return A2 + (int64_t)plan.late[i] * lda2; });
+    if (!left) return;
+    __syncthreads();
+    const double2* t2 = reinterpret_cast<const double2*>(tmp) + b2;
+    move_chunk_rows(
+        plan.npiv[0], lanes, w2, [&](int i, int l) { return t2[(int64_t)i * lda2 + l]; },
+        [&](int i) { return A2 + (int64_t)(fnpr + i) * lda2; });
+}
+
 __global__ void gri_gather_kernel(const int* __restrict__ gri, int* __restrict__ gri_tmp, const int* __restrict__ rowsrc,
                                   int fnpr, int Ml) {
     const int r = fnpr + blockIdx.x * blockDim.x + threadIdx.x;
@@ -312,7 +363,7 @@
 }
 int launch_gather_winners(const double* PT, int64_t ldp, const int* tags, int n_valid, const int* perm, int v,
                           double* out_vals, int64_t ldo, int* out_tags, int dst0, cudaStream_t s) {
-    const int64_t tot = (int64_t)v * v;
+    const int64_t tot = out_vals ? (int64_t)v * v : v;
     gather_winners_kernel<<<(unsigned)((tot + 255) / 256), 256, 0, s>>>(PT, ldp, tags, n_valid, perm, v, out_vals, ldo,
                                                                         out_tags, dst0);
     POST_LAUNCH();
@@ -329,9 +380,25 @@
     POST_LAUNCH();
 }
 int launch_push_phase1(const double* A, int64_t lda, int ncols, int col_lo, MovePlan plan, int v, double* tmp,
-                       double* a01raw, int64_t ld01, int c0, cudaStream_t s) {
+                       double* a01raw, int64_t ld01, int c0, cudaStream_t s, int tmp_hi) {
     dim3 grid(row_chunks(ncols), a01raw ? 2 * v : v);
-    push_phase1_kernel<<<grid, 256, 0, s>>>(A, lda, ncols, col_lo, plan, v, tmp, a01raw, ld01, c0);
+    push_phase1_kernel<<<grid, 256, 0, s>>>(A, lda, ncols, col_lo, tmp_hi < 0 ? ncols : tmp_hi, plan, v, tmp, a01raw, ld01,
+                                            c0);
+    POST_LAUNCH();
+}
+int launch_push_window(double* A, int64_t lda, MovePlan plan, int v, double* a01raw, int64_t ld01, int c0, int w,
+                       cudaStream_t s) {
+    constexpr int lanes = 2;
+    if (w <= 0) return CFLX_OK;
+    push_window_kernel<<<(w / 2 + lanes - 1) / lanes, 256, 0, s>>>(A, lda, plan, v, a01raw, ld01, c0, w, lanes);
+    POST_LAUNCH();
+}
+int launch_push_rest(double* A, int64_t lda, MovePlan plan, int fnpr, const double* tmp, int l_hi, int r_lo, int r_hi,
+                     cudaStream_t s) {
+    constexpr int lanes = 16;
+    const int n = (l_hi / 2 + lanes - 1) / lanes + ((r_hi - r_lo) / 2 + lanes - 1) / lanes;
+    if (n <= 0) return CFLX_OK;
+    push_rest_kernel<<<n, 256, 0, s>>>(A, lda, plan, fnpr, tmp, l_hi, r_lo, r_hi, lanes);
     POST_LAUNCH();
 }
 int launch_push_phase2(double* A, int64_t lda, int ncols, int col_lo, MovePlan plan, int v, cudaStream_t s) {
diff --git a/conflux_b200/csrc/trsm.cu b/conflux_b200/csrc/trsm.cu
--- a/conflux_b200/csrc/trsm.cu
+++ b/conflux_b200/csrc/trsm.cu
@@ -140,6 +140,7 @@
         g.C = nullptr; g.ldc = ld;
         g.D = U + (int64_t)j * nb * ld; g.ldd = ld;
         g.alpha = 1.0; g.beta = 0.0;
+        g.fill_sms = true;
         CFLX_TRY(launch_gemm_tn(g, stream));
         const int rest = v - (j + 1) * nb;
         if (rest > 0) {
@@ -150,6 +151,7 @@
             u.C = R + (int64_t)(j + 1) * nb * ld; u.ldc = ld;
             u.D = R + (int64_t)(j + 1) * nb * ld; u.ldd = ld;
             u.alpha = -1.0; u.beta = 1.0;
+            u.fill_sms = true;
             CFLX_TRY(launch_gemm_tn(u, stream));
         }
     }
diff --git a/include/conflux_b200.h b/include/conflux_b200.h
--- a/include/conflux_b200.h
+++ b/include/conflux_b200.h
@@ -123,6 +123,8 @@
 int cflx_dbg_wgmma_peak(int n, double* tmacs_out);
 int cflx_dbg_push_pivots(int n_rows, int n_cols, double* A_inout, int npiv, const int* pivot_rows, int fnpr, int* gri_out,
                          double* a01_out);
+int cflx_dbg_push_split(int n_rows, int n_cols, double* A_inout, int npiv, const int* pivot_rows, int fnpr, int loff, int c0,
+                        int w, double* a01_out);
 int cflx_dbg_fp64_peak(int which, double* tflops_out);
 int cflx_dbg_fp64_peak_ex(int which, double* burst_out, double* sustained_out);
 
```
